# zhengyk19/vit-rpe-rope

Measured on AMD Instinct MI355X. Metric: train images/sec, CIFAR-10 ViT d=192 L=6 H=6, higher is better.
Workload: dtype bf16; 1 GPU; CIFAR-10-shaped 32x32 patch4 ViT d=192 L=6 H=6, --pos_encoding rope-axial theta=100, bf16, full train step (fwd+CE+bwd+AdamW), random-init weights; per_gpu_batch=512, global_batch=512, parallelism=dp1, hip_graph=True

## Files before the change

include/vitpe.h:

```cpp
#ifndef VITPE_H
#define VITPE_H

#ifdef __cplusplus
extern "C" {
#endif

#define VITPE_F32 0
#define VITPE_BF16 1

#define VITPE_PE_NONE 0
#define VITPE_PE_ABSOLUTE 1
#define VITPE_PE_RELATIVE 2
#define VITPE_PE_POLYNOMIAL 3
#define VITPE_PE_ROPE_AXIAL 4
#define VITPE_PE_ROPE_MIXED 5

#define VITPE_EPI_BIAS 0
#define VITPE_EPI_BIAS_GELU 1
#define VITPE_EPI_BIAS_RESID 2
#define VITPE_EPI_PATCH 3
#define VITPE_EPI_GELU_BWD 4

typedef void* vitpe_stream_t;

int vitpe_abi_version(void);

int vitpe_fused_attention_supported(int dtype, int N, int D, int HD);
int vitpe_pack_qkv_weights(int dtype, const float* wqkv, void* packed, int D, int HD, vitpe_stream_t stream);
int vitpe_fused_attention_fwd(int dtype, const void* xn, const void* wqkv, void* out, int B, int N,
                              int D, int HD, int mode, const float* cos, const float* sin,
                              const float* table, const float* coeff, int grid, int degree,
                              int coeff_per_head, vitpe_stream_t stream);
int vitpe_fused_attention_fwd_ln(int dtype, const void* x, const float* gamma, const float* beta,
                                 const float* mean, const float* rstd, void* xn_out, const void* wqkv,
                                 void* out, int B, int N, int D, int HD, int mode, const float* cos,
                                 const float* sin, const float* table, const float* coeff, int grid,
                                 int degree, int coeff_per_head, vitpe_stream_t stream);
int vitpe_fused_attention_wide_supported(int dtype, int N, int D, int HD);
int vitpe_qkv_wide_pack_elems(int D);
int vitpe_pack_qkv_weights_wide(int dtype, const float* wqkv, void* packed, int D, int HD, vitpe_stream_t stream);
int vitpe_fused_attention_fwd_wide(int dtype, const void* x, const float* gamma, const float* beta,
                                   const float* mean, const float* rstd, void* xn_out, const void* wqkv_wide,
                                   void* out, int B, int N, int D, int HD, int mode, const float* cos,
                                   const float* sin, const float* table, const float* coeff, int grid, int degree,
                                   int coeff_per_head, vitpe_stream_t stream);
int vitpe_fused_attention_bwd(int dtype, const void* xn, const void* wqkv, const void* dout,
                              void* dqkv, int B, int N, int D, int HD, int mode, const float* cos,
                              const float* sin, const float* table, const float* coeff, int grid,
                              int degree, int coeff_per_head, float* dtable, float* dcoeff,
                              float* dfreqs, vitpe_stream_t stream);
int vitpe_fused_attention_bwd_ln(int dtype, const void* x, const float* gamma, const float* beta,
                                 const float* mean, const float* rstd, const void* wqkv, const void* dout,
                                 void* dqkv, int B, int N, int D, int HD, int mode, const float* cos,
                                 const float* sin, const float* table, const float* coeff, int grid,
                                 int degree, int coeff_per_head, float* dtable, float* dcoeff,
                                 float* dfreqs, vitpe_stream_t stream);

int vitpe_attention_core_supported(int dtype, int N, int HD);
int vitpe_attention_core_fwd(int dtype, const void* qkv, void* out, int B, int N, int H, int HD, int mode,
                             const float* cos, const float* sin, const float* table, const float* coeff,
                             int grid, int degree, int coeff_per_head, vitpe_stream_t stream);
int vitpe_attention_core_bwd(int dtype, const void* qkv, const void* dout, void* dqkv, int B, int N, int H,
                             int HD, int mode, const float* cos, const float* sin, const float* table,
                             const float* coeff, int grid, int degree, int coeff_per_head, float* dtable,
                             float* dcoeff, float* dfreqs, vitpe_stream_t stream);
int vitpe_attention_core_bwd_tables(int dtype, const void* qkv, const void* dout, void* dqkv, int B, int N, int H,
                                    int HD, int mode, const float* cos, const float* sin, const float* table,
                                    const float* coeff, int grid, int degree, int coeff_per_head, float* dtable,
                                    float* dcoeff, float* dfreqs, float* dcos, float* dsin, float* workspace,
                                    vitpe_stream_t stream);
int vitpe_attention_fused64_supported(int dtype, int N, int H, int HD);
int vitpe_attention_fused64_fwd(int dtype, const void* xn, const void* wqkv_packed, void* qkv_out, void* out, int B,
                                int N, int H, int HD, int mode, const float* cos, const float* sin,
                                const float* table, const float* coeff, int grid, int degree, int coeff_per_head,
                                vitpe_stream_t stream);

int vitpe_philox4x32_10(const unsigned int* key2, const unsigned int* ctr4, unsigned int* out4);
int vitpe_dropout_mask(int site, const unsigned long long* rng, unsigned char* mask, long long n, int B, int H, int N,
                       float p, vitpe_stream_t stream);
int vitpe_dropout_fwd(int dtype, const void* x, const void* resid, void* y, long long n, const unsigned long long* rng,
                      float p, vitpe_stream_t stream);
int vitpe_dropout_bwd(int dtype, const void* dy, void* dx, long long n, const unsigned long long* rng, float p,
                      vitpe_stream_t stream);
int vitpe_drop_path_fwd(int dtype, const void* x, const void* resid, void* y, int B, long long per,
                        const unsigned long long* rng, float p, vitpe_stream_t stream);
int vitpe_drop_path_bwd(int dtype, const void* dy, void* dx, int B, long long per, const unsigned long long* rng, float p,
                        vitpe_stream_t stream);
int vitpe_attention_core_fwd_drop(int dtype, const void* qkv, void* out, int B, int N, int H, int HD, int mode,
                                  const float* cos, const float* sin, const float* table, const float* coeff,
                                  int grid, int degree, int coeff_per_head, const unsigned long long* rng, float p,
                                  vitpe_stream_t stream);
int vitpe_attention_core_bwd_drop(int dtype, const void* qkv, const void* dout, void* dqkv, int B, int N, int H,
                                  int HD, int mode, const float* cos, const float* sin, const float* table,
                                  const float* coeff, int grid, int degree, int coeff_per_head, float* dtable,
                                  float* dcoeff, float* dfreqs, const unsigned long long* rng, float p,
                                  vitpe_stream_t stream);

int vitpe_gemm_nt(int dtype, int epi, const void* A, const void* W, void* C, const float* bias,
                  const void* R, void* U, const float* ape, const float* cls, int M, int N, int K,
                  int P, int Ntok, vitpe_stream_t stream);
int vitpe_linear(int dtype, int epi, const void* A, const void* W, void* C, const float* bias,
                 const void* R, void* U, float* mean_out, float* rstd_out, float eps, int M, int N,
                 int K, vitpe_stream_t stream);
int vitpe_linear_ln(int dtype, int epi, const void* X, const float* gamma, const float* beta,
                    const float* mean, const float* rstd, void* xn_out, const void* W, void* C,
                    const float* bias, void* U, int M, int N, int K, vitpe_stream_t stream);
int vitpe_linear_lnbwd(int dtype, const void* dY, const void* Wt, void* dx, const void* x, const float* mean,
                       const float* rstd, const float* gamma, const void* dres, float* dgamma, float* dbeta,
                       int M, int K, vitpe_stream_t stream);
int vitpe_linear_lnbwd2(int dtype, const void* dY, const void* Wt_packed, void* dx, const void* x, const float* mean,
                        const float* rstd, const float* gamma, const void* dres, float* dgamma, float* dbeta, int M,
                        int K, vitpe_stream_t stream);
int vitpe_pack_weight_frags(int dtype, const float* W, void* packed, int R, int C, int kchunk, int phi,
                            vitpe_stream_t stream);
int vitpe_block_tail2_supported(int dtype, int D, int HID);
int vitpe_block_tail2_fwd(int dtype, const void* attn_out, const void* x_in, const void* Wp_packed, const float* bp,
                          const float* gamma, const float* beta, void* x_mid, float* mean2, float* rstd2,
                          void* xn_out, const void* W1_packed, const float* b1, const void* W2_packed,
                          const float* b2, void* gp_out, void* h_out, void* out, float* mean_out, float* rstd_out,
                          float eps2, float eps_next, int M, int D, int HID, vitpe_stream_t stream);
int vitpe_block_tail2_bwd(int dtype, const void* dy, const void* gp, const void* W2t_packed, const void* W1t_packed,
                          const void* x_mid, const float* mean2, const float* rstd2, const float* gamma, void* du,
                          void* dx_mid, float* dgamma, float* dbeta, const void* WpT_packed, void* da, int M, int D,
                          int HID, vitpe_stream_t stream);
int vitpe_block_tail2_bwd_pre(int dtype, const void* d_qkv, const void* WqT_packed, const void* x1, const float* mean1,
                              const float* rstd1, const float* gamma1, const void* dres1, float* dgamma1, float* dbeta1,
                              int K1, void* dy_out, const void* gp, const void* W2t_packed, const void* W1t_packed,
                              const void* x_mid, const float* mean2, const float* rstd2, const float* gamma, void* du,
                              void* dx_mid, float* dgamma, float* dbeta, const void* WpT_packed, void* da, int M, int D,
                              int HID, vitpe_stream_t stream);
int vitpe_gemm_tn(int dtype, const void* dY, const void* X, float* dW, float* dbias, int M, int N,
                  int K, int splits, vitpe_stream_t stream);

typedef struct {
  const void* dY;
  const void* X;
  float* dW;
  float* dbias;
  int M, N, K;
  int x_op;
  const float* x_mean;
  const float* x_rstd;
  const float* x_gamma;
  const float* x_beta;
} vitpe_wgrad_problem;
#define VITPE_XOP_NONE 0
#define VITPE_XOP_LAYERNORM 1
int vitpe_wgrad_group(int dtype, const vitpe_wgrad_problem* problems, int nprob, vitpe_stream_t stream);

int vitpe_layernorm_fwd(int dtype, const void* x, const float* gamma, const float* beta, void* y,
                        float* mean, float* rstd, int M, int D, float eps, vitpe_stream_t stream);
int vitpe_layernorm_bwd_blocks(int M);
int vitpe_layernorm_bwd(int dtype, const void* dy, const void* x, const float* mean,
                        const float* rstd, const float* gamma, const void* dres, void* dx,
                        float* dgamma, float* dbeta, float* workspace, int M, int D,
                        vitpe_stream_t stream);
int vitpe_reduce_partials(const float* partial, int nparts, int len0, int len1, float* dst0,
                          float* dst1, vitpe_stream_t stream);

int vitpe_resize_coeffs(int in, int out, int* bounds, int* kk, int ksize_cap);
int vitpe_resize_u8_supported(int S0, int S);
int vitpe_resize_u8(const unsigned char* src, unsigned char* dst, long long planes, int S0, int S,
                    const int* bounds_h, const int* kk_h, const int* bounds_v, const int* kk_v, int ksize,
                    vitpe_stream_t stream);

int vitpe_unfold(int dtype, const float* img, void* patches, int B, int C, int S, int p,
                 vitpe_stream_t stream);
int vitpe_unfold_u8(int dtype, const unsigned char* data, const long long* index, const float* mean,
                    const float* stdv, void* patches, float* img_out, int B, int C, int S, int p,
                    vitpe_stream_t stream);
int vitpe_patch_embed_supported(int dtype, int C, int S, int p, int D);
int vitpe_patch_embed(int dtype, const float* img, const unsigned char* data, const long long* index,
                      const float* nmean, const float* nstd, const void* W, const float* bias, const float* cls,
                      const float* ape, void* tokens, void* patches, float* mean, float* rstd, int B, int C, int S,
                      int p, int D, float eps, vitpe_stream_t stream);
int vitpe_embed_bwd(int dtype, const void* dtok, float* dcls, float* dape, void* dpatch, int B,
                    int Ntok, int D, vitpe_stream_t stream);

int vitpe_relative_position_index(long long* out, int L, vitpe_stream_t stream);
int vitpe_l1_distance_matrix(long long* out, int G, vitpe_stream_t stream);
int vitpe_rope_axial_tables(const float* inv_freq, float* cosv, float* sinv, int G, int half,
                            vitpe_stream_t stream);
int vitpe_rope_mixed_tables(const float* freqs, float* cosv, float* sinv, int H, int G, int half,
                            vitpe_stream_t stream);
int vitpe_relative_bias(const float* table, float* out, int H, int L, vitpe_stream_t stream);
int vitpe_polynomial_bias(const float* coeff, float* out, int H, int G, int degree, int per_head,
                          vitpe_stream_t stream);
int vitpe_relative_bias_bwd(const float* dbias, float* dtable, int H, int L, vitpe_stream_t stream);
int vitpe_polynomial_bias_bwd(const float* dbias, float* dcoeff, int H, int G, int degree, int per_head,
                              vitpe_stream_t stream);
int vitpe_rope_mixed_tables_bwd(const float* freqs, const float* dcos, const float* dsin, float* dfreqs, int H,
                                int G, int half, vitpe_stream_t stream);
int vitpe_apply_rotary(const float* x, float* y, const float* cosv, const float* sinv, int B, int H,
                       int P, int HD, int per_head, vitpe_stream_t stream);
int vitpe_apply_rotary_bwd(const float* dy, const float* x, const float* cosv, const float* sinv, float* dx,
                           float* dcos, float* dsin, float* workspace, int B, int H, int P, int HD, int per_head,
                           vitpe_stream_t stream);

int vitpe_head_fwd(int dtype, const void* x, const float* gamma, const float* beta, const float* Wh,
                   const float* bh, float* logits, float* ws_xhat, float* ws_yn, float* ws_rstd,
                   int B, int Ntok, int D, int Cn, float eps, vitpe_stream_t stream);
int vitpe_cross_entropy(const float* logits, const long long* labels, float* dlogits, float* out2,
                        int B, int Cn, float grad_scale, vitpe_stream_t stream);
int vitpe_cross_entropy_ctl(const float* logits, const long long* labels, float* dlogits, float* out2,
                            float* metric_acc, const float* ctl, int B, int Cn, vitpe_stream_t stream);
int vitpe_head_bwd(int dtype, const float* dlogits, const float* Wh, const float* gamma,
                   const float* ws_xhat, const float* ws_yn, const float* ws_rstd, float* ws_dyn,
                   void* dx, float* dWh, float* dbh, float* dgamma, float* dbeta, int B, int Ntok,
                   int D, int Cn, vitpe_stream_t stream);
int vitpe_head_loss(int dtype, const void* x, const float* gamma, const float* beta, const float* Wh,
                    const float* bh, const long long* labels, float* logits, float* dlogits, float* ws_xhat,
                    float* ws_yn, float* ws_dyn, void* dx, float* out2, float* metric_acc, float* scratch,
                    float* dWh, float* dbh, float* dgamma, float* dbeta, int B, int Ntok, int D, int Cn,
                    float eps, float grad_scale, vitpe_stream_t stream);

int vitpe_head_step(int dtype, const void* x, const float* gamma, const float* beta, const float* Wh,
                    const float* bh, const long long* labels, float* logits, float* dlogits, float* ws_xhat,
                    float* ws_yn, float* ws_dyn, void* dx, float* out2, float* metric_acc, float* per_image,
                    const float* ctl, float* dWh, float* dbh, float* dgamma, float* dbeta, int B, int Ntok,
                    int D, int Cn, float eps, float* hp_tick, vitpe_stream_t stream);

int vitpe_adamw_step(float* p, float* g, float* m, float* v, void* shadow_bf16, float* hp,
                     long long n, int zero_grad, vitpe_stream_t stream);
int vitpe_cast(int dtype, const float* src, void* dst, long long n, vitpe_stream_t stream);
int vitpe_transpose_cast(int dtype, const float* src, void* dst, int R, int C, vitpe_stream_t stream);
int vitpe_refresh_shadows(int dtype, const float* flat, void* dst_base, const void* desc, int ndesc,
                          int total_tiles, const unsigned short* tile_map, vitpe_stream_t stream);


#ifdef __cplusplus
}
#endif
#endif
```

vit-rpe-rope_amd/csrc/wgrad.hip:

```cpp
#include "common.h"
#include <stdlib.h>

namespace vitpe {

constexpr int WG_MAXPROB = 28;
constexpr int WG_BLK = 192;

struct WgProb {
  const void* dY;
  const void* X;
  float* dW;
  float* dbias;
  const float* xmean;
  const float* xrstd;
  const float* xgamma;
  const float* xbeta;
  int M, N, K;
  int xop;
  int unit0;
  int nbn;
  int stages;
};
constexpr int WG_TABLE = 512;
struct WgArgs {
  int nprob, total_units, units_per_wg;
  int use_table;
  int nranges;
  int full_rounds, total_blocks;
  int tail_rounds;
  int bk;
  int range_major;
  unsigned long long* census;
  WgProb p[WG_MAXPROB];
  unsigned short table[WG_TABLE];
};
static_assert(sizeof(WgArgs) <= 4096, "kernel argument block");
constexpr int WG_CENSUS_STAGES = 24, WG_CENSUS_SLOTS = 4;

template <typename T> struct WgLayout;
template <> struct WgLayout<bf16> {
  static constexpr int LD = WG_BLK;
  static __device__ __forceinline__ int chunk(int r, int cc) {
    const int s = ((r >> 1) & 1) | (((r >> 3) & 1) << 1);
    return r * LD + ((((cc >> 1) ^ s)) << 4) + ((cc & 1) << 3);
  }
  static __device__ __forceinline__ Frag<bf16> tr(const bf16* tile, int rb0, int rb1, int c0) { return tr_ld<LD>(tile, rb0, rb1, c0); }
  template <int LD>
  static __device__ __forceinline__ Frag<bf16> tr_ld(const bf16* tile, int rb0, int rb1, int c0) {
    const int i = threadIdx.x & 15, q = i >> 2, p = i & 3;
    typedef __attribute__((address_space(3))) s16x4 lds_s16x4;
    const int r0 = rb0 + q, r1 = rb1 + q;
    constexpr int PAR = (LD % 128 == 0) ? 4 : 0;
    const int s0 = (((r0 >> 1) & 1) | (((r0 >> 3) & 1) << 1)) ^ ((r0 & 1) * PAR), s1 = (((r1 >> 1) & 1) | (((r1 >> 3) & 1) << 1)) ^ ((r1 & 1) * PAR);
    const bf16* a0 = tile + r0 * LD + (((c0 >> 4) ^ s0) << 4) + 4 * p;
    const bf16* a1 = tile + r1 * LD + (((c0 >> 4) ^ s1) << 4) + 4 * p;
    s16x4 lo = __builtin_amdgcn_ds_read_tr16_b64_v4i16((lds_s16x4*)a0);
    s16x4 hi = __builtin_amdgcn_ds_read_tr16_b64_v4i16((lds_s16x4*)a1);
    const s16x8 both = __builtin_shufflevector(lo, hi, 0, 1, 2, 3, 4, 5, 6, 7);
    Frag<bf16> f;
    f.v = __builtin_bit_cast(bf16x8, both);
    return f;
  }
};
template <> struct WgLayout<float> {
  static constexpr int LD = WG_BLK + 4;
  static __device__ __forceinline__ int chunk(int r, int cc) { return r * LD + cc * 4; }
  static __device__ __forceinline__ Frag<float> tr(const float* tile, int rb0, int rb1, int c0) {
    return ld_frag_tr(tile, LD, rb0, rb1, c0);
  }
};

template <class RunFn>
VITPE_DEV void wg_dispatch(const WgArgs& a, RunFn run) {
  if (a.use_table == 2) {
    const int G = gridDim.x, idx = (blockIdx.x & 7) * (G >> 3) + (blockIdx.x >> 3);
    const int nrounds = a.range_major ? a.full_rounds : a.full_rounds + a.tail_rounds;
    for (int r = 0; r < nrounds; ++r) {
      int gb, rng = 0, R = 1;
      if (a.range_major) {
        const int vb = r * G + idx;
        R = a.nranges;
        rng = vb / a.total_blocks;
        gb = rng < R ? vb - rng * a.total_blocks : a.total_blocks;
      } else if (r < a.full_rounds) {
        gb = r * G + idx;
      } else {
        R = a.nranges;
        const int rem = a.total_blocks - a.full_rounds * G, q = (r - a.full_rounds) * G + idx;
        if (q >= rem * R) continue;
        rng = q / rem;
        gb = a.full_rounds * G + q % rem;
      }
      if (gb >= a.total_blocks) continue;
      int pi = 0, b0 = 0;
      for (int i = 0; i < a.nprob; ++i) {
        const int nb = a.p[i].nbn * ((a.p[i].K + a.bk - 1) / a.bk);
        if (gb >= b0 + nb) { b0 += nb; pi = i + 1; } else break;
      }
      const WgProb& P = a.p[pi];
      const int spr = (P.stages + R - 1) / R;
      const int ub = P.unit0 + (gb - b0) * P.stages;
      const int u0 = ub + min(P.stages, rng * spr), uend = ub + min(P.stages, (rng + 1) * spr);
      if (u0 < uend) run(u0, uend);
    }
    return;
  }
  int u0, uend;
  if (a.use_table == 1) {
    const unsigned ent = a.table[blockIdx.x];
    if (ent == 0xFFFFu) return;
    const WgProb& P = a.p[ent >> 11];
    const int blk = (int)((ent >> 5) & 0x3Fu), rng = (int)(ent & 0x1Fu);
    const int spr = (P.stages + a.nranges - 1) / a.nranges;
    u0 = P.unit0 + blk * P.stages + min(P.stages, rng * spr);
    uend = P.unit0 + blk * P.stages + min(P.stages, (rng + 1) * spr);
  } else {
    u0 = blockIdx.x * a.units_per_wg;
    uend = min(a.total_units, u0 + a.units_per_wg);
  }
  if (u0 >= uend) return;
  run(u0, uend);
}

template <typename T, bool CENSUS, bool LNX>
__global__ __launch_bounds__(768) void wgrad_group_kernel(WgArgs a) {
  using LY = WgLayout<T>;
  constexpr int RPS = 128 / (int)sizeof(T);
  constexpr int CPS = RPS / 32;
  constexpr int CHN = CH<T>::n;
  constexpr int CPR = WG_BLK / CHN;
  static_assert(RPS * CPR == 2 * 768, "a slab is two chunks per thread");
  constexpr int SLAB = RPS * LY::LD;
  __shared__ __attribute__((aligned(16))) T sm[2 * 2 * SLAB];

  const int tid = threadIdx.x, lane = tid & 63, c = lane & 15, g = lane >> 4;
  const int wave = __builtin_amdgcn_readfirstlane(tid >> 6);
  const int wn = wave / 3, wk = wave % 3;

  struct Cur {
    const T* dY; const T* X; float* dW; float* dbias;
    const float* xmean; const float* xrstd; const float* xgamma; const float* xbeta;
    int M, N, K, n0, k0, stage, stages, xop;
  };
  auto decode = [&](int u, Cur& s) {
    int pi = 0;
    for (int i = 1; i < a.nprob; ++i) pi = (u >= a.p[i].unit0) ? i : pi;
    const WgProb& P = a.p[pi];
    const int ub = u - P.unit0, blk = ub / P.stages;
    s.dY = reinterpret_cast<const T*>(P.dY); s.X = reinterpret_cast<const T*>(P.X); s.dW = P.dW; s.dbias = P.dbias;
    s.M = P.M; s.N = P.N; s.K = P.K; s.stages = P.stages;
    s.xmean = P.xop ? P.xmean : reinterpret_cast<const float*>(P.dY);
    s.xrstd = P.xop ? P.xrstd : reinterpret_cast<const float*>(P.dY);
    s.xgamma = P.xgamma; s.xbeta = P.xbeta; s.xop = P.xop;
    s.stage = ub - blk * P.stages;
    s.n0 = (blk % P.nbn) * WG_BLK;
    s.k0 = (blk / P.nbn) * a.bk;
  };

  const Chunk16 zero = {0u, 0u, 0u, 0u};
  Chunk16 rg[4];
  float lnA[2], lnB[2];
  bool ln_staged = false;
  auto gload = [&](const Cur& s) {
    const int mb = s.stage * RPS;
    ln_staged = LNX && s.xop == 1;
#pragma unroll
    for (int i = 0; i < 4; ++i) {
      const int q = tid + 768 * (i & 1), row = q / CPR, cc = q % CPR;
      const int gm = mb + row;
      if (i < 2) {
        const int gn = s.n0 + cc * CHN;
        rg[i] = (gm < s.M && gn < s.N) ? *reinterpret_cast<const Chunk16*>(s.dY + (size_t)gm * s.N + gn) : zero;
      } else {
        const int gk = s.k0 + cc * CHN;
        const bool ok = gm < s.M && gk < s.K;
        rg[i] = ok ? *reinterpret_cast<const Chunk16*>(s.X + (size_t)gm * s.K + gk) : zero;
        if (LNX) {
          const int gs = (s.xop == 1) ? min(gm, s.M - 1) : 0;
          lnA[i - 2] = s.xrstd[gs];
          lnB[i - 2] = s.xmean[gs];
        }
      }
    }
  };
  auto sstore = [&](int buf) {
#pragma unroll
    for (int i = 0; i < 4; ++i) {
      const int q = tid + 768 * (i & 1), row = q / CPR, cc = q % CPR;
      Chunk16 v = rg[i];
      if (LNX && i >= 2 && ln_staged) {
        float f[CHN];
        chunk_to_f32<T>(v, f);
        const float rs = lnA[i - 2], nb = -lnB[i - 2] * rs;
#pragma unroll
        for (int t = 0; t < CHN; ++t) f[t] = fmaf(f[t], rs, nb);
        v = f32_to_chunk<T>(f);
      }
      *reinterpret_cast<Chunk16*>(sm + (buf * 2 + (i >> 1)) * SLAB + LY::chunk(row, cc)) = v;
    }
  };

  f32x4 acc[3][4], accb[3];
  auto clear = [&]() {
#pragma unroll
    for (int nt = 0; nt < 3; ++nt) {
      accb[nt] = (f32x4){0.f, 0.f, 0.f, 0.f};
#pragma unroll
      for (int kt = 0; kt < 4; ++kt) acc[nt][kt] = (f32x4){0.f, 0.f, 0.f, 0.f};
    }
  };
  Frag<T> ones;
#pragma unroll
  for (int t = 0; t < 8; ++t) ones.v[t] = from_f32<T>(1.0f);

  auto compute = [&](int buf, bool bias) {
    const T* sY = sm + (buf * 2 + 0) * SLAB;
    const T* sX = sm + (buf * 2 + 1) * SLAB;
#pragma unroll
    for (int cs = 0; cs < CPS; ++cs) {
      const int rb0 = cs * 32 + 8 * g, rb1 = rb0 + 4;
      Frag<T> fy[3], fx[4];
#pragma unroll
      for (int nt = 0; nt < 3; ++nt) fy[nt] = LY::tr(sY, rb0, rb1, wn * 48 + 16 * nt);
#pragma unroll
      for (int kt = 0; kt < 4; ++kt) fx[kt] = LY::tr(sX, rb0, rb1, wk * 64 + 16 * kt);
#pragma unroll
      for (int nt = 0; nt < 3; ++nt)
#pragma unroll
        for (int kt = 0; kt < 4; ++kt) mma(fy[nt], fx[kt], acc[nt][kt]);
      if (bias) {
#pragma unroll
        for (int nt = 0; nt < 3; ++nt) mma(fy[nt], ones, accb[nt]);
      }
    }
  };
  auto flush = [&](const Cur& s, bool bias) {
    float gam[4], bet[4];
#pragma unroll
    for (int kt = 0; kt < 4; ++kt) {
      const int gk = s.k0 + wk * 64 + 16 * kt + c;
      gam[kt] = (LNX && s.xop == 1 && gk < s.K) ? s.xgamma[gk] : 1.f;
      bet[kt] = (LNX && s.xop == 1 && gk < s.K) ? s.xbeta[gk] : 0.f;
    }
#pragma unroll
    for (int nt = 0; nt < 3; ++nt)
#pragma unroll
      for (int r = 0; r < 4; ++r) {
        const int gn = s.n0 + wn * 48 + 16 * nt + 4 * g + r;
#pragma unroll
        for (int kt = 0; kt < 4; ++kt) {
          const int gk = s.k0 + wk * 64 + 16 * kt + c;
          float v = acc[nt][kt][r];
          if (LNX && s.xop == 1) v = fmaf(v, gam[kt], bet[kt] * accb[nt][r]);
          if (gn < s.N && gk < s.K) atomicAdd(s.dW + (size_t)gn * s.K + gk, v);
        }
        if (bias && c == 0 && gn < s.N) atomicAdd(s.dbias + gn, accb[nt][r]);
      }
    clear();
  };

  bool first_run = true;
  auto run = [&](int u0, int uend) {
    if (!first_run) __syncthreads();
    first_run = false;
  Cur cur, nxt;
    decode(u0, cur);
    gload(cur);
    clear();
    auto stamp = [&](int u, int slot) {
      if (CENSUS && lane == 0 && u - u0 < WG_CENSUS_STAGES)
        a.census[(((size_t)blockIdx.x * 12 + wave) * WG_CENSUS_STAGES + (u - u0)) * WG_CENSUS_SLOTS + slot] = __builtin_amdgcn_s_memtime();
    };
    for (int u = u0; u < uend; ++u) {
      const int buf = (u - u0) & 1;
      sstore(buf);
      stamp(u, 0);
      nxt = cur;
      bool flush_now = (u + 1 == uend);
      if (u + 1 < uend) {
        if (cur.stage + 1 < cur.stages) nxt.stage = cur.stage + 1;
        else { decode(u + 1, nxt); flush_now = true; }
        gload(nxt);
      }
      stamp(u, 2);
      __syncthreads();
      stamp(u, 1);
      const bool bias = (cur.dbias != nullptr) && cur.k0 == 0 && wk == 0;
      compute(buf, bias || (LNX && cur.xop == 1));
      stamp(u, 3);
      if (flush_now) flush(cur, bias);
      cur = nxt;
    }
  };

  wg_dispatch(a, run);
}

constexpr int WW_BK = 384, WW_TH = 512;

__global__ __launch_bounds__(WW_TH) void wgrad_wide_kernel(WgArgs a) {
  using T = bf16;
  using LY = WgLayout<bf16>;
  constexpr int RPS = 64, YLD = WG_BLK, XLD = WW_BK;
  constexpr int YSLAB = RPS * YLD, XSLAB = RPS * XLD, STG = YSLAB + XSLAB;
  constexpr int YI = YSLAB / 512, XI = XSLAB / 512, NI = (YI + XI) / 8;
  static_assert((YI + XI) % 8 == 0, "instructions per wave");
  __shared__ __attribute__((aligned(1024))) T sm[2 * STG];

  const int tid = threadIdx.x, lane = tid & 63, c = lane & 15, g = lane >> 4;
  const int wave = __builtin_amdgcn_readfirstlane(tid >> 6);
  const int wn = wave >> 2, wk = wave & 3;

  struct Cur { const T* dY; const T* X; float* dW; float* dbias; int M, N, K, n0, k0, stage, stages; };
  auto decode = [&](int u, Cur& s) {
    int pi = 0;
    for (int i = 1; i < a.nprob; ++i) pi = (u >= a.p[i].unit0) ? i : pi;
    const WgProb& P = a.p[pi];
    const int ub = u - P.unit0, blk = ub / P.stages;
    s.dY = reinterpret_cast<const T*>(P.dY); s.X = reinterpret_cast<const T*>(P.X); s.dW = P.dW; s.dbias = P.dbias;
    s.M = P.M; s.N = P.N; s.K = P.K; s.stages = P.stages;
    s.stage = ub - blk * P.stages;
    s.n0 = (blk % P.nbn) * WG_BLK;
    s.k0 = (blk / P.nbn) * WW_BK;
  };
  auto swz = [](int r, int cl) { return ((((cl >> 1) ^ (((r >> 1) & 1) | (((r >> 3) & 1) << 1))) << 1) | (cl & 1)); };
  auto swzx = [](int r, int cl) {
    return ((((cl >> 1) ^ ((((r >> 1) & 1) | (((r >> 3) & 1) << 1)) ^ ((r & 1) << 2))) << 1) | (cl & 1));
  };
  static_assert(YI == 24 && XI == 48, "instruction j of a wave: j < 3 -> dY slab, else X slab");
  const unsigned sm_lds = (unsigned)(uintptr_t)(__attribute__((address_space(3))) void*)sm;
  auto dma = [&](const Cur& s, int buf) {
    const int mb = s.stage * RPS;
    int ln = lane;
    asm volatile("" : "+v"(ln));
#pragma unroll
    for (int j = 0; j < NI; ++j) {
      const int q = wave + 8 * j;
      const T* src;
      if (j < 3) {
        const int p = q * 64 + ln, r = p / (YLD / 8), cl = p % (YLD / 8);
        src = s.dY + (size_t)min(mb + r, s.M - 1) * s.N + s.n0 + swz(r, cl) * 8;
      } else {
        const int p = (q - YI) * 64 + ln, r = p / (XLD / 8), cl = p % (XLD / 8);
        src = s.X + (size_t)min(mb + r, s.M - 1) * s.K + s.k0 + swzx(r, cl) * 8;
      }
      const unsigned dst = sm_lds + (unsigned)(buf * STG + q * 512) * 2;
      unsigned keep;
      asm volatile("s_mov_b32 %0, m0\n\ts_mov_b32 m0, %2\n\ts_nop 0\n\tglobal_load_lds_dwordx4 %1, off\n\ts_mov_b32 m0, %0"
                   : "=&s"(keep) : "v"(src), "s"(dst) : "memory");
    }
  };

  f32x4 acc[6][6], accb[2];
  auto clear = [&]() {
    accb[0] = accb[1] = (f32x4){0.f, 0.f, 0.f, 0.f};
#pragma unroll
    for (int nt = 0; nt < 6; ++nt)
#pragma unroll
      for (int kt = 0; kt < 6; ++kt) acc[nt][kt] = (f32x4){0.f, 0.f, 0.f, 0.f};
  };
  Frag<T> ones;
#pragma unroll
  for (int t = 0; t < 8; ++t) ones.v[t] = from_f32<T>(1.0f);

  auto compute = [&](int buf, bool bias) {
    const T* sY = sm + buf * STG;
    const T* sX = sY + YSLAB;
#pragma unroll
    for (int cs = 0; cs < 2; ++cs) {
      const int rb0 = cs * 32 + 8 * g, rb1 = rb0 + 4;
      __builtin_amdgcn_sched_barrier(0);
      Frag<T> fy[6];
#pragma unroll
      for (int nt = 0; nt < 6; ++nt) fy[nt] = LY::tr_ld<YLD>(sY, rb0, rb1, wn * 96 + 16 * nt);
#pragma unroll
      for (int h = 0; h < 2; ++h) {
        Frag<T> fx[3];
#pragma unroll
        for (int t = 0; t < 3; ++t) fx[t] = LY::tr_ld<XLD>(sX, rb0, rb1, wk * 96 + 16 * (3 * h + t));
#pragma unroll
        for (int nt = 0; nt < 6; ++nt)
#pragma unroll
          for (int t = 0; t < 3; ++t) mma(fy[nt], fx[t], acc[nt][3 * h + t]);
        __builtin_amdgcn_sched_barrier(0);
      }
      if (bias) {
        if (wk == 0) { mma(fy[0], ones, accb[0]); mma(fy[1], ones, accb[1]); }
        else if (wk == 1) { mma(fy[2], ones, accb[0]); mma(fy[3], ones, accb[1]); }
        else { mma(fy[4], ones, accb[0]); mma(fy[5], ones, accb[1]); }
      }
    }
  };
  auto flush = [&](const Cur& s, bool bias) {
#pragma unroll
    for (int nt = 0; nt < 6; ++nt)
#pragma unroll
      for (int r = 0; r < 4; ++r) {
        const int gn = s.n0 + wn * 96 + 16 * nt + 4 * g + r;
        float* row = s.dW + (size_t)gn * s.K + s.k0 + wk * 96 + c;
#pragma unroll
        for (int kt = 0; kt < 6; ++kt) atomicAdd(row + 16 * kt, acc[nt][kt][r]);
      }
    if (bias && c == 0) {
#pragma unroll
      for (int t = 0; t < 2; ++t)
#pragma unroll
        for (int r = 0; r < 4; ++r) atomicAdd(s.dbias + s.n0 + wn * 96 + 16 * (2 * wk + t) + 4 * g + r, accb[t][r]);
    }
    clear();
  };

  bool first_run = true;
  auto run = [&](int u0, int uend) {
    if (!first_run) __syncthreads();
    first_run = false;
    Cur cur, nxt;
    decode(u0, cur);
    dma(cur, 0);
    clear();
    for (int u = u0; u < uend; ++u) {
      const int buf = (u - u0) & 1;
      __builtin_amdgcn_s_waitcnt(0x0F70);
      __syncthreads();
      if (cur.stage * RPS + RPS > cur.M) {
        const int first = cur.M - cur.stage * RPS;
        T* sY = sm + buf * STG;
        for (int q = tid; q < (RPS - first) * (YLD / 8); q += WW_TH)
          *reinterpret_cast<Chunk16*>(sY + first * YLD + q * 8) = (Chunk16){0u, 0u, 0u, 0u};
        __syncthreads();
      }
      nxt = cur;
      bool flush_now = (u + 1 == uend);
      if (u + 1 < uend) {
        if (cur.stage + 1 < cur.stages) nxt.stage = cur.stage + 1;
        else { decode(u + 1, nxt); flush_now = true; }
        dma(nxt, buf ^ 1);
      }
      const bool bias = (cur.dbias != nullptr) && cur.k0 == 0 && wk < 3;
      compute(buf, bias);
      if (flush_now) flush(cur, bias);
      cur = nxt;
    }
  };
  wg_dispatch(a, run);
}

}

using namespace vitpe;

struct vitpe_wgrad_problem_abi {
  const void* dY;
  const void* X;
  float* dW;
  float* dbias;
  int M, N, K, x_op;
  const float* x_mean;
  const float* x_rstd;
  const float* x_gamma;
  const float* x_beta;
};

static int wgrad_cu_count() {
  static int n = 0;
  if (n == 0) {
    int dev = 0, v = 0;
    if (hipGetDevice(&dev) != hipSuccess || hipDeviceGetAttribute(&v, hipDeviceAttributeMultiprocessorCount, dev) != hipSuccess || v <= 0)
      v = 256;
    n = v;
  }
  return n;
}

static int wgrad_group_launch(int dtype, const void* problems, int nprob, unsigned long long* census, hipStream_t stream);
static bool g_wide_ok = true;
extern "C" int vitpe_debug_set_wgrad_wide(int on) { g_wide_ok = on != 0; return 0; }

extern "C" int vitpe_wgrad_group(int dtype, const void* problems, int nprob, hipStream_t stream) {
  return wgrad_group_launch(dtype, problems, nprob, nullptr, stream);
}

extern "C" int vitpe_debug_wgrad_census(int dtype, const void* problems, int nprob, unsigned long long* census,
                                        hipStream_t stream) {
  VITPE_REQUIRE(census != nullptr && dtype == 1);
  return wgrad_group_launch(dtype, problems, nprob, census, stream);
}

static int wgrad_group_launch(int dtype, const void* problems, int nprob, unsigned long long* census, hipStream_t stream) {
  VITPE_REQUIRE(problems && nprob >= 0 && nprob <= WG_MAXPROB && (dtype == 0 || dtype == 1));
  const vitpe_wgrad_problem_abi* pr = reinterpret_cast<const vitpe_wgrad_problem_abi*>(problems);
  const int RPS = dtype == 1 ? 64 : 32, CHN = dtype == 1 ? 8 : 4;
  WgArgs a{};
  a.census = census;
  bool wide = g_wide_ok && dtype == 1 && census == nullptr && nprob > 0;
  for (int i = 0; i < nprob; ++i)
    wide = wide && (pr[i].M == 0 || (pr[i].x_op == 0 && pr[i].N % WG_BLK == 0 && pr[i].K % WW_BK == 0));
  a.bk = wide ? WW_BK : WG_BLK;
  int units = 0, np = 0;
  for (int i = 0; i < nprob; ++i) {
    const vitpe_wgrad_problem_abi& p = pr[i];
    VITPE_REQUIRE(p.dY && p.X && p.dW && p.M >= 0 && p.N > 0 && p.K > 0 && p.N % CHN == 0 && p.K % CHN == 0);
    if (p.M == 0) continue;
    WgProb& q = a.p[np++];
    VITPE_REQUIRE(p.x_op == 0 || (p.x_op == 1 && p.x_mean && p.x_rstd && p.x_gamma && p.x_beta));
    q.dY = p.dY; q.X = p.X; q.dW = p.dW; q.dbias = p.dbias; q.M = p.M; q.N = p.N; q.K = p.K;
    q.xop = p.x_op; q.xmean = p.x_mean; q.xrstd = p.x_rstd; q.xgamma = p.x_gamma; q.xbeta = p.x_beta;
    q.unit0 = units;
    q.nbn = (p.N + WG_BLK - 1) / WG_BLK;
    q.stages = (p.M + RPS - 1) / RPS;
    const long long nu = (long long)q.nbn * ((p.K + a.bk - 1) / a.bk) * q.stages;
    VITPE_REQUIRE(units + nu < (1LL << 30));
    units += (int)nu;
  }
  if (units == 0) return 0;
  a.nprob = np;
  a.total_units = units;
  const int ncu = wgrad_cu_count();
  int grid = 0;
  int total_blocks = 0, max_blocks = 0, min_stages = 1 << 30;
  for (int i = 0; i < np; ++i) {
    const int nb = a.p[i].nbn * ((a.p[i].K + a.bk - 1) / a.bk);
    total_blocks += nb;
    max_blocks = nb > max_blocks ? nb : max_blocks;
    min_stages = a.p[i].stages < min_stages ? a.p[i].stages : min_stages;
  }
  int R = (2 * ncu) / (total_blocks > 0 ? total_blocks : 1);
  if (R > 255) R = 255;
  if (R >= 2 && R <= 8 && R <= min_stages / 4 && max_blocks <= 63 && np <= 31) {
    int len[8] = {0, 0, 0, 0, 0, 0, 0, 0};
    bool fits = true;
    for (int i = 0; i < WG_TABLE; ++i) a.table[i] = 0xFFFFu;
    for (int r = 0; r < R && fits; ++r)
      for (int i = 0; i < np && fits; ++i) {
        const int nb = a.p[i].nbn * ((a.p[i].K + a.bk - 1) / a.bk);
        int x = 0;
        for (int k = 1; k < 8; ++k) x = len[k] < len[x] ? k : x;
        for (int b = 0; b < nb; ++b) {
          const int id = (len[x] + b) * 8 + x;
          if (id >= WG_TABLE) { fits = false; break; }
          a.table[id] = (unsigned short)(((unsigned)i << 11) | ((unsigned)b << 5) | (unsigned)r);
        }
        len[x] += nb;
      }
    if (fits) {
      int mx = 0;
      for (int k = 0; k < 8; ++k) mx = len[k] > mx ? len[k] : mx;
      a.use_table = 1;
      a.nranges = R;
      grid = mx * 8;
    }
  }
  const int G = ncu & ~7;
  if (!a.use_table && G >= 8 && total_blocks >= G) {
    a.use_table = 2;
    a.total_blocks = total_blocks;
    a.full_rounds = total_blocks / G;
    const int rem = total_blocks - a.full_rounds * G;
    int bestR = 1, bestT = rem > 0 ? 1 : 0;
    int Rmax = min_stages / 4;
    if (Rmax > 8) Rmax = 8;
    for (int Rc = 2; rem > 0 && Rc <= Rmax; ++Rc) {
      const int Tc = (rem * Rc + G - 1) / G;
      if ((long long)Tc * bestR < (long long)bestT * Rc) { bestR = Rc; bestT = Tc; }
    }
    a.nranges = bestR;
    a.tail_rounds = bestT;
    grid = G;
  }
  if (!a.use_table && G >= 8 && total_blocks > 0 && total_blocks < G) {
    int bestR = 0, bestk = 0;
    double besteff = 0.0;
    for (int k = 1; k <= 3; ++k) {
      int Rk = (k * G) / total_blocks;
      if (Rk > min_stages / 4) Rk = min_stages / 4;
      if (Rk > 31) Rk = 31;
      if (Rk < 2) continue;
      const double eff = (double)total_blocks * Rk / (double)(((total_blocks * Rk + G - 1) / G) * G);
      if (eff > besteff + 1e-9) { besteff = eff; bestR = Rk; bestk = k; }
    }
    if (bestR >= 2 && besteff >= 0.97) {
      a.use_table = 2;
      a.range_major = 1;
      a.total_blocks = total_blocks;
      a.nranges = bestR;
      a.full_rounds = (total_blocks * bestR + G - 1) / G;
      grid = G;
      (void)bestk;
    }
  }
  if (!a.use_table) {
    const int wgs = units < ncu ? units : ncu;
    a.units_per_wg = (units + wgs - 1) / wgs;
    grid = (units + a.units_per_wg - 1) / a.units_per_wg;
  }
  bool lnx = false;
  for (int i = 0; i < np; ++i) lnx = lnx || a.p[i].xop != 0;
  if (census != nullptr) VITPE_REQUIRE(!lnx && dtype == 1);
  if (wide) hipLaunchKernelGGL(wgrad_wide_kernel, dim3(grid), dim3(WW_TH), 0, stream, a);
  else if (census != nullptr) hipLaunchKernelGGL((wgrad_group_kernel<bf16, true, false>), dim3(grid), dim3(768), 0, stream, a);
  else if (dtype == 1 && lnx) hipLaunchKernelGGL((wgrad_group_kernel<bf16, false, true>), dim3(grid), dim3(768), 0, stream, a);
  else if (dtype == 1) hipLaunchKernelGGL((wgrad_group_kernel<bf16, false, false>), dim3(grid), dim3(768), 0, stream, a);
  else if (lnx) hipLaunchKernelGGL((wgrad_group_kernel<float, false, true>), dim3(grid), dim3(768), 0, stream, a);
  else hipLaunchKernelGGL((wgrad_group_kernel<float, false, false>), dim3(grid), dim3(768), 0, stream, a);
  VITPE_CHECK_LAUNCH();
}
```

vit-rpe-rope_amd/vitpe/engine.py:

```python
from __future__ import annotations

import math
import os
from typing import Dict, List, Optional

import torch
import torch.distributed as dist
import torch.nn as nn

from . import _lib as L
from . import ddp
from . import kernels as K
from .positional_encoding import (AbsolutePositionalEncoding, PolynomialRPE, RelativePositionalEncoding, RoPEAxial,
                                  RoPEMixed)
from .vit import VisionTransformer

ALIGN = 8


def engine_unsupported(model):
    active = []
    for blk in model.blocks:
        if blk.attn.qkv.bias is not None:
            active.append("qkv_bias")
        if blk.attn.attn_drop_p > 0.:
            active.append("attn_drop")
        if blk.attn.proj_drop_p > 0. or blk.mlp.drop > 0.:
            active.append("drop")
        if blk.drop_path_p > 0.:
            active.append("drop_path")
    return sorted(set(active))


class TrainEngine:
    def __init__(self, model: VisionTransformer, batch_size: int, compute_dtype=torch.bfloat16, lr=1e-3,
                 weight_decay=0.01, betas=(0.9, 0.999), eps=1e-8, process_group=None, use_graph=True, fuse_ln=None):
        active = engine_unsupported(model)
        if active:
            raise NotImplementedError("TrainEngine does not support " + ", ".join(active) + " (the fused training path has "
                                      "no qkv bias and no dropout); train this model through the module path instead")
        dev = next(model.parameters()).device
        if dev.type != "cuda":
            raise L.VitpeError("TrainEngine needs the model on the HIP device (no CPU path)")
        self.model, self.dev, self.T, self.B = model, dev, compute_dtype, batch_size
        self.pg = process_group
        self.world = dist.get_world_size(process_group) if (dist.is_available() and dist.is_initialized()) else 1
        self.use_graph = use_graph
        m = model
        ok = m.embed_dim == 192
        if fuse_ln is None and "VITPE_FUSE_LN" in os.environ:
            fuse_ln = {"fwd": "fwd", "all": True, "off": False}[os.environ["VITPE_FUSE_LN"]]
        self.fuse_ln = ok and fuse_ln is not False
        self.fuse_ln_bwd = ok and (fuse_ln is True or fuse_ln is None)
        self.D, self.H, self.Lyr = m.embed_dim, m.num_heads, len(m.blocks)
        self.p = m.patch_size
        self.C = m.patch_embed.weight.shape[1]

        self.P = m.num_patches
        self.N = self.P + 1
        self.grid = int(math.sqrt(self.P))
        self.S = self.grid * self.p
        self.fuse_embed = (os.environ.get("VITPE_FUSE_EMBED", "1") == "1" and
                           K.patch_embed_supported(compute_dtype, self.C, self.S, self.p, self.D))
        self.hid = m.blocks[0].mlp.fc1.weight.shape[0]
        self.Cn = m.num_classes
        self.M = self.B * self.N
        self.attn_fused = K.fused_attention_supported(self.T, self.N, self.D, self.D // self.H)
        if not self.attn_fused and not K.attention_core_supported(self.T, self.N, self.D // self.H):
            raise L.VitpeError(f"no attention kernel for N={self.N}, D={self.D}, hd={self.D // self.H}")
        self._save_hidden = True
        self.attn_wide = (self.attn_fused and K.fused_attention_wide_supported(self.T, self.N, self.D, self.D // self.H)
                          and os.environ.get("VITPE_ATTN_WIDE", "1") == "1")
        self.attn_fused64 = (not self.attn_fused and os.environ.get("VITPE_ATTN_FUSED64", "1") == "1"
                             and K.attention_fused64_supported(self.T, self.N, self.H, self.D // self.H))
        if not self.attn_fused:
            self.fuse_ln = self.fuse_ln_bwd = False
        self.tail2 = (self.fuse_ln and self.fuse_ln_bwd and os.environ.get("VITPE_TAIL2", "1") == "1"
                      and K.block_tail2_supported(self.T, self.D, self.hid))
        self.lnbwd2 = self.tail2 and os.environ.get("VITPE_LNBWD2", "1") == "1"
        self.fuse_lnbwd = self.lnbwd2 and os.environ.get("VITPE_FUSE_LNBWD", "1") == "1"
        self._build_flat(lr, weight_decay, betas, eps)
        self._build_buffers()
        self.split_layer = max(1, self.Lyr // 2)
        self.bucket_off = self._off[id(next(self.model.blocks[self.split_layer].parameters()))] \
            if self.Lyr >= 2 else 0
        self.overlap_comm = self.world > 1 and self.Lyr >= 2
        self.allpairs = (ddp.AllPairsSum(self.pg) if self.world > 1 and os.environ.get("VITPE_DDP_ALLPAIRS", "0") == "1"
                         else None)
        self._comm_stream = torch.cuda.Stream(device=dev) if self.allpairs is not None else None
        self.ddp_graph = self.world > 1 and os.environ.get("VITPE_DDP_GRAPH", "0") == "1"
        self.graph_fb = self.graph_fb2 = self.graph_opt = None
        self.steps_done = 0

    def _build_flat(self, lr, wd, betas, eps):
        params = list(self.model.parameters())
        starts, n = ddp.flat_layout([prm.numel() for prm in params], ALIGN)
        offs = {id(prm): o for prm, o in zip(params, starts)}
        self.n_flat = n
        f = dict(dtype=torch.float32, device=self.dev)
        self.flat_p, self.flat_g = torch.zeros(n, **f), torch.zeros(n, **f)
        self.flat_m, self.flat_v = torch.zeros(n, **f), torch.zeros(n, **f)
        self.flat_s = torch.zeros(n, dtype=torch.bfloat16, device=self.dev) if self.T == torch.bfloat16 else None
        self._off = offs
        for prm in params:
            o = offs[id(prm)]
            view = self.flat_p[o:o + prm.numel()].view(prm.shape)
            view.copy_(prm.data)
            prm.data = view
            prm.grad = self.flat_g[o:o + prm.numel()].view(prm.shape)
        self.model.register_load_state_dict_post_hook(lambda _m, _keys: self.sync_from_model())
        self.hp = torch.zeros(16, **f)
        self.hp[:5] = torch.tensor([lr, betas[0], betas[1], eps, wd], **f)
        self.hp[8] = 1.0 / self.world
        self._st: Dict[int, torch.Tensor] = {}
        self._pk: Dict[int, torch.Tensor] = {}
        self._pkw: Dict[int, torch.Tensor] = {}
        self._fr: Dict[int, torch.Tensor] = {}
        self._frt: Dict[int, torch.Tensor] = {}
        self._gemm_weights: List[nn.Parameter] = []
        recs, off, tile0 = [], 0, 0
        def alloc(w):
            nonlocal off
            o = off
            off += (w.numel() + ALIGN - 1) // ALIGN * ALIGN
            return o
        def add(w, kind, hd, kind2=-1, hd2=0):
            nonlocal tile0
            R, C = w.shape
            o1 = alloc(w)
            o2 = alloc(w) if kind2 >= 0 else 0
            recs.append((self._off[id(w)], o1, o2, R, C, tile0, kind, hd, kind2, hd2, 0))
            tile0 += ((R + 31) // 32) * ((C + 31) // 32)
            spans.append((w, kind, o1))
            if kind2 >= 0:
                spans.append((w, kind2, o2))
        spans = []
        HDh = self.D // self.H
        gen2 = self.tail2
        for blk in self.model.blocks:
            qkv, proj, fc1, fc2 = blk.attn.qkv.weight, blk.attn.proj.weight, blk.mlp.fc1.weight, blk.mlp.fc2.weight
            self._gemm_weights += [qkv, proj, fc1, fc2]
            if self.attn_fused:
                add(qkv, 1, HDh, *((4, 64) if self.lnbwd2 else (0, 0)))
                if self.attn_wide:
                    add(qkv, 6, HDh)
            else:
                add(qkv, 0, 0, *((2, 64) if self.attn_fused64 else ()))
            if self.tail2:
                add(proj, 2, 192, *((5, 192) if gen2 else (0, 0)))
                add(fc1, 3, 192, *((5, 32) if gen2 else (0, 0)))
                add(fc2, 3, 32, *((5, 192) if gen2 else (0, 0)))
            else:
                for w in (proj, fc1, fc2):
                    add(w, 0, 0)
        self._shadow_flat = torch.empty(off, dtype=self.T, device=self.dev)
        for w, kind, o in spans:
            R, C = w.shape
            if kind == 0:
                self._st[id(w)] = self._shadow_flat[o:o + R * C].view(C, R)
            elif kind == 1:
                self._pk[id(w)] = self._shadow_flat[o:o + R * C].view(R, C)
            elif kind == 6:
                self._pkw[id(w)] = self._shadow_flat[o:o + R * C]
            elif kind < 4:
                self._fr[id(w)] = self._shadow_flat[o:o + R * C].view(R, C)
            else:
                self._frt[id(w)] = self._shadow_flat[o:o + R * C].view(C, R)
        import numpy as np
        rec = np.zeros(len(recs), dtype=np.dtype([("src", "<i8"), ("dst", "<i8"), ("dst2", "<i8"), ("R", "<i4"), ("C", "<i4"),
                                                   ("tile0", "<i4"), ("kind", "<i4"), ("HD", "<i4"), ("kind2", "<i4"),
                                                   ("HD2", "<i4"), ("pad", "<i4")]))
        for i, r in enumerate(recs):
            rec[i] = r
        self._desc = torch.from_numpy(rec.view(np.uint8).copy()).to(self.dev)
        self._ndesc, self._ntiles = len(recs), tile0
        tmap = np.zeros(tile0, dtype=np.int16)
        for i, r in enumerate(recs):
            tmap[r[5]:] = i
        self._tile_map = torch.from_numpy(tmap).to(self.dev)
        self.refresh_shadows()

    def Pm(self, prm):
        return prm.data

    def Gr(self, prm):
        o = self._off[id(prm)]
        return self.flat_g[o:o + prm.numel()].view(prm.shape)

    def Sh(self, prm):
        if self.T == torch.float32:
            return prm.data
        o = self._off[id(prm)]
        return self.flat_s[o:o + prm.numel()].view(prm.shape)

    def St(self, prm):
        return self._st[id(prm)]

    def Pk(self, prm):
        return self._pk[id(prm)]

    def Pkw(self, prm):
        return self._pkw[id(prm)]

    def _attn_fwd(self, x, blk, out, ln=None, xn_out=None):
        if self.attn_wide:
            return K.fused_attention_fwd_wide(x, self.Pkw(blk.attn.qkv.weight), self.H, self.pe, out=out, ln=ln, xn_out=xn_out)
        return K.fused_attention_fwd(x, self.Pk(blk.attn.qkv.weight), self.H, self.pe, out=out, ln=ln, xn_out=xn_out)

    def _attn_layer_fwd(self, l, save_qkv=True):
        blk, a = self.model.blocks[l], self.act[l]
        if self.fuse_ln:
            return self._attn_fwd(self.x[l], blk, a["a"], ln=(blk.norm1.weight.data, blk.norm1.bias.data, a["m1"], a["r1"]),
                                  xn_out=a["xn1"])
        if self.attn_fused:
            return self._attn_fwd(a["xn1"], blk, a["a"])
        if self.attn_fused64:
            return K.attention_fused64_fwd(a["xn1"], self.Fr(blk.attn.qkv.weight), self.H, self.pe,
                                           qkv_out=(self.qkv_l[l] if save_qkv else None), out=a["a"])
        return K.attention_core_fwd(self.qkv_l[l], self.H, self.pe, out=a["a"])

    def _attn_bwd(self, l, dout):
        blk, a = self.model.blocks[l], self.act[l]
        if not self.attn_fused:
            return K.attention_core_bwd(self.qkv_l[l], dout, self.H, self.pe, out=self.dqkv_l[l], **self.pe_grads)
        if self.recompute_ln:
            return K.fused_attention_bwd(self.x[l], self.Pk(blk.attn.qkv.weight), dout, self.H, self.pe, out=self.dqkv_l[l],
                                         ln=(blk.norm1.weight.data, blk.norm1.bias.data, a["m1"], a["r1"]), **self.pe_grads)
        return K.fused_attention_bwd(a["xn1"], self.Pk(blk.attn.qkv.weight), dout, self.H, self.pe, out=self.dqkv_l[l],
                                     **self.pe_grads)

    def Fr(self, prm):
        return self._fr[id(prm)]

    def Frt(self, prm):
        return self._frt[id(prm)]

    def refresh_shadows(self, cast_flat=True):
        if self.T == torch.bfloat16 and cast_flat:
            K.cast(self.flat_p, torch.bfloat16, out=self.flat_s)
        K.refresh_shadows(self.flat_p, self._shadow_flat, self._desc, self._ndesc, self._ntiles, self._tile_map)

    def set_lr(self, lr: float):
        self.hp[0] = lr

    def _build_buffers(self):
        B, N, D, M, T, dev = self.B, self.N, self.D, self.M, self.T, self.dev
        e = lambda *s, dt=T: torch.empty(*s, dtype=dt, device=dev)
        f = lambda *s: torch.empty(*s, dtype=torch.float32, device=dev)
        self.images = f(B, self.C, self.S, self.S)
        self.labels = torch.zeros(B, dtype=torch.int64, device=dev)
        self.patches = e(B * self.P, self.C * self.p * self.p)
        self.x = [e(B, N, D) for _ in range(self.Lyr + 1)]
        self.group_wgrad = os.environ.get("VITPE_GROUP_WGRAD", "1") == "1"
        self.recompute_ln = (self.attn_fused and self.fuse_ln and self.fuse_ln_bwd and self.tail2
                             and self.group_wgrad and os.environ.get("VITPE_RECOMPUTE_LN", "0") == "1")
        xn = (lambda: None) if self.recompute_ln else (lambda: e(B, N, D))
        self.act = []
        for _ in range(self.Lyr):
            self.act.append(dict(xn1=xn(), m1=f(M), r1=f(M), a=e(B, N, D), xmid=e(B, N, D), xn2=xn(),
                                 m2=f(M), r2=f(M), h=e(M, self.hid), u=e(M, self.hid)))
        self.logits, self.dlogits = f(B, self.Cn), f(B, self.Cn)
        self.out2 = f(2)
        self.metric_acc = torch.zeros(2, dtype=torch.float32, device=dev)
        self.ce_ctl = torch.zeros(4, dtype=torch.float32, device=dev)
        self._valid = None
        self.set_valid(B)
        self.head_scratch = torch.zeros(2 * B, dtype=torch.float32, device=dev)
        self.fuse_head = self.Cn <= 64 and self.D <= 768 and os.environ.get("VITPE_FUSE_HEAD", "1") == "1"
        self.head_ws = (f(B, D), f(B, D), f(B))
        self.ws_dyn = f(B, D)
        self.dtmp = e(B, N, D)
        self.dx_out = [e(B, N, D) for _ in range(self.Lyr + 1)]
        self.dx_out[self.Lyr].zero_()
        self.dx_mid = [e(B, N, D) for _ in range(self.Lyr)]
        self.du_l = [e(M, self.hid) for _ in range(self.Lyr)]
        self.dqkv_l = [e(B, N, 3 * D) for _ in range(self.Lyr)]
        self.qkv_l = [] if self.attn_fused else [e(B, N, 3 * D) for _ in range(self.Lyr)]
        self.dqkv, self.du = self.dqkv_l[0], self.du_l[0]
        self.dataset, self.batch_idx = None, None
        self._wg_groups = {}
        self.dpatch = e(B * self.P, D)
        self.ln_ws = K.layernorm_bwd_workspace(M, D, dev)
        pe = self.model.pos_embed
        mode = self.model.pos_encoding_type
        self.pe = K.PETables(mode if mode != "absolute" else "none", self.grid)
        self.pe_grads = dict(dtable=None, dcoeff=None, dfreqs=None)
        if isinstance(pe, RelativePositionalEncoding):
            self.pe.table = pe.relative_position_bias_table.data
            self.pe_grads["dtable"] = self.Gr(pe.relative_position_bias_table)
        elif isinstance(pe, PolynomialRPE):
            self.pe.coeff, self.pe.degree = pe.coefficients.data, pe.degree
            self.pe.coeff_per_head = not pe.shared_across_heads
            self.pe_grads["dcoeff"] = self.Gr(pe.coefficients)
        elif isinstance(pe, RoPEAxial):
            self.pe.cos, self.pe.sin = K.rope_axial_tables(pe.inv_freq.contiguous(), self.grid)
        elif isinstance(pe, RoPEMixed):
            self.pe.cos, self.pe.sin = K.rope_mixed_tables(pe.freqs.data, self.grid)
            self.pe_grads["dfreqs"] = self.Gr(pe.freqs)

    def _forward(self, head=True, save=False):
        self._save_hidden = save
        mdl, B, N, D, M = self.model, self.B, self.N, self.D, self.M
        ape = mdl.pos_embed.pos_embed.data[0, :self.P] if isinstance(mdl.pos_embed, AbsolutePositionalEncoding) else None
        if self.fuse_embed:
            src = (dict(data=self.dataset.images, index=self.batch_idx, mean=self.dataset.mean, std=self.dataset.std)
                   if self.dataset is not None else dict(images=self.images))
            b0 = mdl.blocks[0]
            K.patch_embed(self.Sh(mdl.patch_embed.weight).view(D, -1), mdl.patch_embed.bias.data, mdl.cls_token.data.view(-1),
                          ape, self.p, self.T, out=self.x[0], patches_out=self.patches,
                          stats=(self.act[0]["m1"], self.act[0]["r1"]) if self.fuse_ln else None, eps=b0.norm1.eps, **src)
        else:
            if self.dataset is not None:
                K.unfold_u8(self.dataset.images, self.batch_idx, self.dataset.mean, self.dataset.std, self.p, self.T,
                            out=self.patches)
            else:
                K.unfold(self.images, self.p, self.T, out=self.patches)
            K.patch_embed_gemm(self.patches, self.Sh(mdl.patch_embed.weight).view(D, -1), mdl.patch_embed.bias.data,
                               mdl.cls_token.data.view(-1), ape, B, self.P, out=self.x[0])
            if self.fuse_ln:
                b0 = mdl.blocks[0]
                K.layernorm_fwd(self.x[0], b0.norm1.weight.data, b0.norm1.bias.data, b0.norm1.eps, mean=self.act[0]["m1"],
                                rstd=self.act[0]["r1"], stats_only=True)
        if isinstance(mdl.pos_embed, RoPEMixed):
            K.rope_mixed_tables(mdl.pos_embed.freqs.data, self.grid, self.pe.cos, self.pe.sin)
        for l, blk in enumerate(mdl.blocks):
            a, xin = self.act[l], self.x[l]
            if self.fuse_ln:
                self._attn_layer_fwd(l)
                nxt = (self.act[l + 1]["m1"], self.act[l + 1]["r1"]) if l + 1 < self.Lyr else None
                eps_next = mdl.blocks[min(l + 1, self.Lyr - 1)].norm1.eps
                if self.tail2:
                    self._block_tail_fwd(l, blk, a, nxt)
                    continue
                K.linear(a["a"].view(M, D), self.Sh(blk.attn.proj.weight), blk.attn.proj.bias.data,
                         epi=L.EPI_BIAS_RESID, resid=xin.view(M, D), out=a["xmid"].view(M, D), stats=(a["m2"], a["r2"]),
                         eps=blk.norm2.eps)
                K.linear_ln(a["xmid"].view(M, D), blk.norm2.weight.data, blk.norm2.bias.data, a["m2"], a["r2"],
                            self.Sh(blk.mlp.fc1.weight), blk.mlp.fc1.bias.data, epi=L.EPI_BIAS_GELU, u=a["u"], out=a["h"],
                            xn_out=a["xn2"].view(M, D))
                K.linear(a["h"], self.Sh(blk.mlp.fc2.weight), blk.mlp.fc2.bias.data, epi=L.EPI_BIAS_RESID,
                         resid=a["xmid"].view(M, D), out=self.x[l + 1].view(M, D), stats=nxt, eps=eps_next)
                continue
            K.layernorm_fwd(xin, blk.norm1.weight.data, blk.norm1.bias.data, blk.norm1.eps, out=a["xn1"],
                            mean=a["m1"], rstd=a["r1"])
            if not self.attn_fused and not self.attn_fused64:
                K.linear(a["xn1"].view(M, D), self.Sh(blk.attn.qkv.weight), None, out=self.qkv_l[l].view(M, 3 * D))
            self._attn_layer_fwd(l, save_qkv=self._save_hidden)
            K.linear(a["a"].view(M, D), self.Sh(blk.attn.proj.weight), blk.attn.proj.bias.data, epi=L.EPI_BIAS_RESID,
                     resid=xin.view(M, D), out=a["xmid"].view(M, D))
            K.layernorm_fwd(a["xmid"], blk.norm2.weight.data, blk.norm2.bias.data, blk.norm2.eps, out=a["xn2"],
                            mean=a["m2"], rstd=a["r2"])
            K.linear(a["xn2"].view(M, D), self.Sh(blk.mlp.fc1.weight), blk.mlp.fc1.bias.data, epi=L.EPI_BIAS_GELU,
                     u=a["u"], out=a["h"])
            K.linear(a["h"], self.Sh(blk.mlp.fc2.weight), blk.mlp.fc2.bias.data, epi=L.EPI_BIAS_RESID,
                     resid=a["xmid"].view(M, D), out=self.x[l + 1].view(M, D))
        if head:
            K.head_fwd(self.x[-1], mdl.norm.weight.data, mdl.norm.bias.data, mdl.head.weight.data, mdl.head.bias.data,
                       mdl.norm.eps, save=True, logits=self.logits, ws=self.head_ws)

    def _block_tail_fwd(self, l, blk, a, nxt, save=None):
        M, D = self.M, self.D
        eps_next = self.model.blocks[min(l + 1, self.Lyr - 1)].norm1.eps
        if save is None:
            save = self._save_hidden
        K.block_tail2_fwd(a["a"].view(M, D), self.x[l].view(M, D), self.Fr(blk.attn.proj.weight),
                          blk.attn.proj.bias.data, blk.norm2.weight.data, blk.norm2.bias.data,
                          self.Fr(blk.mlp.fc1.weight), blk.mlp.fc1.bias.data, self.Fr(blk.mlp.fc2.weight),
                          blk.mlp.fc2.bias.data, x_mid=a["xmid"].view(M, D), mean2=a["m2"], rstd2=a["r2"],
                          xn_out=(a["xn2"].view(M, D) if (save and not self.recompute_ln) else None),
                          gp=(a["u"].view(torch.float16) if save else None), h=(a["h"] if save else None), out=self.x[l + 1].view(M, D),
                          stats=nxt, eps2=blk.norm2.eps, eps_next=eps_next, save=save)

    def _block_tail_bwd(self, l, blk, a, pre=False):
        M, D, G = self.M, self.D, self.Gr
        if pre:
            up, ua = self.model.blocks[l + 1], self.act[l + 1]
            K.block_tail2_bwd_pre(self.dqkv_l[l + 1].view(M, 3 * D), self.Frt(up.attn.qkv.weight), self.x[l + 1].view(M, D),
                                  ua["m1"], ua["r1"], up.norm1.weight.data, self.dx_mid[l + 1].view(M, D), G(up.norm1.weight),
                                  G(up.norm1.bias), self.dx_out[l + 1].view(M, D), a["u"].view(torch.float16), self.Frt(blk.mlp.fc2.weight),
                                  self.Frt(blk.mlp.fc1.weight), a["xmid"].view(M, D), a["m2"], a["r2"], blk.norm2.weight.data,
                                  G(blk.norm2.weight), G(blk.norm2.bias), self.Frt(blk.attn.proj.weight), du=self.du_l[l],
                                  out=self.dx_mid[l].view(M, D), da=self.dtmp.view(M, D))
            return
        K.block_tail2_bwd(self.dx_out[l + 1].view(M, D), a["u"].view(torch.float16), self.Frt(blk.mlp.fc2.weight),
                          self.Frt(blk.mlp.fc1.weight), a["xmid"].view(M, D), a["m2"], a["r2"], blk.norm2.weight.data,
                          G(blk.norm2.weight), G(blk.norm2.bias), self.Frt(blk.attn.proj.weight), du=self.du_l[l],
                          out=self.dx_mid[l].view(M, D), da=self.dtmp.view(M, D))

    def _tail_bytes(self, fwd: bool) -> int:
        M, D, hid, es = self.M, self.D, self.hid, 2 if self.T == torch.bfloat16 else 4
        if fwd:
            return ((4 if self.recompute_ln else 5) * M * D + 2 * M * hid) * es
        return (4 * M * D + 2 * M * hid) * es

    def _fwd_train(self):
        self._forward(head=not self.fuse_head, save=True)

    def _loss(self, tick=True):
        self._ticked = bool(tick and self.fuse_head)
        if self.fuse_head:
            mdl, G = self.model, self.Gr
            K.head_step(self.x[-1], mdl.norm.weight.data, mdl.norm.bias.data, mdl.head.weight.data, mdl.head.bias.data,
                        self.labels, self.logits, self.dlogits, self.head_ws, self.ws_dyn, self.dx_out[self.Lyr], self.out2,
                        self.metric_acc, self.head_scratch, self.ce_ctl, G(mdl.head.weight), G(mdl.head.bias),
                        G(mdl.norm.weight), G(mdl.norm.bias), eps=mdl.norm.eps, hp_tick=(self.hp if tick else None))
            return
        K.cross_entropy_ctl(self.logits, self.labels, self.ce_ctl, dlogits=self.dlogits, out2=self.out2,
                            metric_acc=self.metric_acc)

    def _wgrad_problems(self, lo, hi, with_embed):
        mdl, D, M, G = self.model, self.D, self.M, self.Gr
        probs = []
        for l in range(hi, lo - 1, -1):
            blk, a = mdl.blocks[l], self.act[l]
            if self.recompute_ln:
                fc1 = (self.du_l[l], a["xmid"].view(M, D), G(blk.mlp.fc1.weight), G(blk.mlp.fc1.bias),
                       (a["m2"], a["r2"], blk.norm2.weight.data, blk.norm2.bias.data))
                qkv = (self.dqkv_l[l].view(M, 3 * D), self.x[l].view(M, D), G(blk.attn.qkv.weight), None,
                       (a["m1"], a["r1"], blk.norm1.weight.data, blk.norm1.bias.data))
            else:
                fc1 = (self.du_l[l], a["xn2"].view(M, D), G(blk.mlp.fc1.weight), G(blk.mlp.fc1.bias))
                qkv = (self.dqkv_l[l].view(M, 3 * D), a["xn1"].view(M, D), G(blk.attn.qkv.weight), None)
            probs += [(self.dx_out[l + 1].view(M, D), a["h"], G(blk.mlp.fc2.weight), G(blk.mlp.fc2.bias)), fc1,
                      (self.dx_mid[l].view(M, D), a["a"].view(M, D), G(blk.attn.proj.weight), G(blk.attn.proj.bias)), qkv]
        if with_embed:
            probs.append((self.dpatch, self.patches, G(mdl.patch_embed.weight).view(D, -1), G(mdl.patch_embed.bias)))
        return probs

    def _wgrad_group(self, part):
        if part not in self._wg_groups:
            hi, lo = self.Lyr - 1, 0
            if part == "upper":
                lo = self.split_layer
            elif part == "lower":
                hi = self.split_layer - 1
            probs = self._wgrad_problems(lo, hi, part != "upper")
            ng = -(-len(probs) // K.WgradGroup.MAX)
            per = -(-len(probs) // ng)
            self._wg_groups[part] = [K.WgradGroup(probs[i:i + per]) for i in range(0, len(probs), per)]
        for grp in self._wg_groups[part]:
            grp.launch()

    def _wgrad(self, fn):
        if not self.group_wgrad:
            fn()

    def _backward(self, part="all"):
        mdl, B, N, D, M = self.model, self.B, self.N, self.D, self.M
        G = self.Gr
        hi, lo = self.Lyr - 1, 0
        if part == "upper":
            lo = self.split_layer
        elif part == "lower":
            hi = self.split_layer - 1
        if part != "lower" and not self.fuse_head:
            dxL = self.dx_out[self.Lyr]
            K.head_bwd(self.dlogits, mdl.head.weight.data, mdl.norm.weight.data, self.head_ws, self.T, N,
                       G(mdl.head.weight), G(mdl.head.bias), G(mdl.norm.weight), G(mdl.norm.bias), dx=dxL,
                       ws_dyn=self.ws_dyn)
        for l in range(hi, lo - 1, -1):
            blk, a = mdl.blocks[l], self.act[l]
            dy3, dmid3, du, dqkv = self.dx_out[l + 1], self.dx_mid[l], self.du_l[l], self.dqkv_l[l]
            dy = dy3.view(M, D)
            self._wgrad(lambda: K.gemm_tn(dy, a["h"], G(blk.mlp.fc2.weight), G(blk.mlp.fc2.bias)))
            fc1_wgrad = lambda: K.gemm_tn(du, a["xn2"].view(M, D), G(blk.mlp.fc1.weight), G(blk.mlp.fc1.bias))
            tail_done = False
            if self.tail2:
                self._block_tail_bwd(l, blk, a, pre=(self.fuse_lnbwd and self.group_wgrad and l < hi))
                self._wgrad(fc1_wgrad)
                tail_done = True
            else:
                K.linear(dy, self.St(blk.mlp.fc2.weight), None, epi=L.EPI_GELU_BWD, u=a["u"], out=du)
                self._wgrad(fc1_wgrad)
                if self.fuse_ln_bwd:
                    K.linear_lnbwd(du, self.St(blk.mlp.fc1.weight), a["xmid"].view(M, D), a["m2"], a["r2"],
                                   blk.norm2.weight.data, dy, G(blk.norm2.weight), G(blk.norm2.bias),
                                   out=dmid3.view(M, D))
                else:
                    K.linear(du, self.St(blk.mlp.fc1.weight), None, out=self.dtmp.view(M, D))
                    K.layernorm_bwd(self.dtmp, a["xmid"], a["m2"], a["r2"], blk.norm2.weight.data, G(blk.norm2.weight),
                                    G(blk.norm2.bias), dres=dy3, out=dmid3, workspace=self.ln_ws)
            dm = dmid3.view(M, D)
            self._wgrad(lambda: K.gemm_tn(dm, a["a"].view(M, D), G(blk.attn.proj.weight), G(blk.attn.proj.bias)))
            if not tail_done:
                K.linear(dm, self.St(blk.attn.proj.weight), None, out=self.dtmp.view(M, D))
            self._attn_bwd(l, self.dtmp)
            self._wgrad(lambda: K.gemm_tn(dqkv.view(M, 3 * D), a["xn1"].view(M, D), G(blk.attn.qkv.weight), None))
            if self.fuse_lnbwd and self.group_wgrad and l > lo:
                pass
            elif self.fuse_ln_bwd and self.lnbwd2:
                K.linear_lnbwd2(dqkv.view(M, 3 * D), self.Frt(blk.attn.qkv.weight), self.x[l].view(M, D), a["m1"],
                                a["r1"], blk.norm1.weight.data, dm, G(blk.norm1.weight), G(blk.norm1.bias),
                                out=self.dx_out[l].view(M, D))
            elif self.fuse_ln_bwd:
                K.linear_lnbwd(dqkv.view(M, 3 * D), self.St(blk.attn.qkv.weight), self.x[l].view(M, D), a["m1"],
                               a["r1"], blk.norm1.weight.data, dm, G(blk.norm1.weight), G(blk.norm1.bias),
                               out=self.dx_out[l].view(M, D))
            else:
                K.linear(dqkv.view(M, 3 * D), self.St(blk.attn.qkv.weight), None, out=self.dtmp.view(M, D))
                K.layernorm_bwd(self.dtmp, self.x[l], a["m1"], a["r1"], blk.norm1.weight.data, G(blk.norm1.weight),
                                G(blk.norm1.bias), dres=dmid3, out=self.dx_out[l], workspace=self.ln_ws)
        if part != "upper":
            dape = None
            if isinstance(mdl.pos_embed, AbsolutePositionalEncoding):
                dape = G(mdl.pos_embed.pos_embed)[0, :self.P]
            K.embed_bwd(self.dx_out[0], G(mdl.cls_token).view(-1), dape, out=self.dpatch)
            if not self.group_wgrad:
                K.gemm_tn(self.dpatch, self.patches, G(mdl.patch_embed.weight).view(D, -1), G(mdl.patch_embed.bias))
        if self.group_wgrad:
            self._wgrad_group(part)

    def _optimizer(self):
        K.adamw_step(self.flat_p, self.flat_g, self.flat_m, self.flat_v, self.hp, shadow_bf16=self.flat_s, ticked=getattr(self, "_ticked", False),
                     zero_grad=True)
        self._ticked = False
        self.refresh_shadows(cast_flat=False)

    def _allreduce(self):
        if self.allpairs is not None:
            self.allpairs(self.flat_g)
        else:
            ddp.allreduce_sum_(self.flat_g, self.pg)

    def set_valid(self, n_valid: int, n_valid_global: Optional[int] = None):
        if n_valid_global is None:
            n_valid_global = n_valid * self.world
        if not (0 <= n_valid <= self.B and n_valid_global >= max(n_valid, 1)):
            raise L.VitpeError(f"set_valid({n_valid}, {n_valid_global}) with engine batch {self.B}")
        if self._valid != (n_valid, n_valid_global):
            self._valid = (n_valid, n_valid_global)
            host = torch.tensor([self.world / n_valid_global, 1.0 / n_valid_global, float(n_valid), 0.0])
            self.ce_ctl.copy_(host, non_blocking=False)

    def sync_from_model(self):
        self.refresh_shadows()

    def broadcast_parameters(self, src=0):
        if self.world > 1:
            ddp.broadcast_(self.flat_p, src, self.pg)
            self.refresh_shadows()

    def capture(self):
        snap = [t.clone() for t in (self.flat_p, self.flat_m, self.flat_v, self.hp, self.metric_acc)]
        s = torch.cuda.Stream()
        s.wait_stream(torch.cuda.current_stream())
        with torch.cuda.stream(s):
            for _ in range(2):
                self._fwd_train(); self._loss(); self._backward(); self._optimizer()
        torch.cuda.current_stream().wait_stream(s)
        torch.cuda.synchronize()
        for t, c in zip((self.flat_p, self.flat_m, self.flat_v, self.hp, self.metric_acc), snap):
            t.copy_(c)
        self.flat_g.zero_()
        self.refresh_shadows()
        torch.cuda.synchronize()
        if self.ddp_graph:
            try:
                g = torch.cuda.CUDAGraph()
                with torch.cuda.graph(g, capture_error_mode="thread_local"):
                    self._fwd_train(); self._loss()
                    if self.overlap_comm:
                        self._backward("upper")
                        side, main = torch.cuda.Stream(), torch.cuda.current_stream()
                        side.wait_stream(main)
                        with torch.cuda.stream(side):
                            dist.all_reduce(self.flat_g[self.bucket_off:], op=dist.ReduceOp.SUM, group=self.pg)
                        self._backward("lower")
                        dist.all_reduce(self.flat_g[:self.bucket_off], op=dist.ReduceOp.SUM, group=self.pg)
                        main.wait_stream(side)
                    else:
                        self._backward()
                        self._allreduce()
                    self._optimizer()
                torch.cuda.synchronize()
                self.graph_fb, self.graph_fb2, self.graph_opt = g, None, None
                return
            except Exception as exc:
                import warnings
                warnings.warn(f"VITPE_DDP_GRAPH: capturing the all-reduces failed ({exc!r}); using the host-stitched step")
                self.ddp_graph = False
                torch.cuda.synchronize()
                self.flat_g.zero_()
        self.graph_fb = torch.cuda.CUDAGraph()
        with torch.cuda.graph(self.graph_fb, capture_error_mode="thread_local"):
            self._fwd_train(); self._loss()
            if self.world == 1:
                self._backward(); self._optimizer()
            elif self.overlap_comm:
                self._backward("upper")
            else:
                self._backward()
        if self.world > 1:
            if self.overlap_comm:
                self.graph_fb2 = torch.cuda.CUDAGraph()
                with torch.cuda.graph(self.graph_fb2, capture_error_mode="thread_local"):
                    self._backward("lower")
            self.graph_opt = torch.cuda.CUDAGraph()
            with torch.cuda.graph(self.graph_opt, capture_error_mode="thread_local"):
                self._optimizer()
        torch.cuda.synchronize()

    def attach_dataset(self, dataset):
        if dataset is self.dataset:
            return
        if dataset is not None:
            C, S = dataset.images.shape[1], dataset.images.shape[2]
            if (C, S) != (self.C, self.S) or dataset.images.device != self.dev:
                raise L.VitpeError(f"dataset is {C}x{S}x{S} on {dataset.images.device}, engine expects "
                                   f"{self.C}x{self.S}x{self.S} on {self.dev}")
            if self.batch_idx is None:
                self.batch_idx = torch.zeros(self.B, dtype=torch.int64, device=self.dev)
        self.dataset = dataset
        self.graph_fb = self.graph_fb2 = self.graph_opt = None

    def _load_indices(self, idx: torch.Tensor, dataset=None):
        dataset = dataset if dataset is not None else self.dataset
        if dataset is None:
            raise L.VitpeError("no dataset attached (TrainEngine.attach_dataset)")
        n = idx.shape[0] if idx.dim() == 1 else -1
        if not (1 <= n <= self.B) or idx.dtype != torch.int64:
            raise L.VitpeError(f"expected 1..{self.B} int64 sample indices, got {tuple(idx.shape)} {idx.dtype}")
        if n < self.B:
            self.batch_idx.fill_(idx[0])
            self.batch_idx[:n].copy_(idx, non_blocking=True)
        else:
            self.batch_idx.copy_(idx, non_blocking=True)
        torch.index_select(dataset.labels, 0, self.batch_idx, out=self.labels)
        return n

    def step_indexed(self, idx: torch.Tensor, n_valid_global: Optional[int] = None, n_valid: Optional[int] = None):
        n = self._load_indices(idx)
        self.set_valid(n if n_valid is None else min(n, n_valid), n_valid_global)
        self.step()

    def forward_indexed(self, idx: torch.Tensor, dataset=None) -> torch.Tensor:
        keep = self.dataset
        if dataset is not None:
            if self.batch_idx is None:
                self.batch_idx = torch.zeros(self.B, dtype=torch.int64, device=self.dev)
            self.dataset = dataset
        try:
            n = self._load_indices(idx)
            self._forward()
        finally:
            self.dataset = keep
        return self.logits[:n]

    def _load_batch(self, images, labels):
        n = images.shape[0]
        if not (1 <= n <= self.B) or tuple(images.shape[1:]) != tuple(self.images.shape[1:]):
            raise L.VitpeError(f"engine was built for batches of up to {self.B} x {tuple(self.images.shape[1:])}, "
                               f"got {tuple(images.shape)}")
        if n < self.B:
            self.images.copy_(images[:1].expand_as(self.images))
            self.images[:n].copy_(images, non_blocking=True)
            if labels is not None:
                self.labels.fill_(0)
                self.labels[:n].copy_(labels, non_blocking=True)
        else:
            self.images.copy_(images, non_blocking=True)
            if labels is not None:
                self.labels.copy_(labels, non_blocking=True)
        return n

    def step(self, images: Optional[torch.Tensor] = None, labels: Optional[torch.Tensor] = None,
             n_valid_global: Optional[int] = None, exchange: bool = True):
        if images is not None:
            if self.dataset is not None:
                raise L.VitpeError("a resident dataset is attached: use step_indexed (or attach_dataset(None))")
            self.set_valid(self._load_batch(images, labels), n_valid_global)
        if self.use_graph:
            if self.graph_fb is None:
                self.capture()
            self.graph_fb.replay()
            if self.world > 1 and not self.ddp_graph:
                if self.overlap_comm:
                    w1 = w2 = None
                    if exchange and self.allpairs is not None:
                        main = torch.cuda.current_stream()
                        self._comm_stream.wait_stream(main)
                        with torch.cuda.stream(self._comm_stream):
                            self.allpairs(self.flat_g[self.bucket_off:])
                        self.graph_fb2.replay()
                        self.allpairs(self.flat_g[:self.bucket_off])
                        main.wait_stream(self._comm_stream)
                        self.graph_opt.replay()
                        self.steps_done += 1
                        return
                    if exchange:
                        w1 = dist.all_reduce(self.flat_g[self.bucket_off:], op=dist.ReduceOp.SUM, group=self.pg, async_op=True)
                    self.graph_fb2.replay()
                    if exchange:
                        w2 = dist.all_reduce(self.flat_g[:self.bucket_off], op=dist.ReduceOp.SUM, group=self.pg, async_op=True)
                        w1.wait(); w2.wait()
                elif exchange:
                    self._allreduce()
                self.graph_opt.replay()
        else:
            self._fwd_train(); self._loss(); self._backward()
            if exchange:
                self._allreduce()
            self._optimizer()
        self.steps_done += 1

    def forward_backward(self):
        self._fwd_train(); self._loss(tick=False); self._backward()

    def forward_only(self, images: torch.Tensor, labels: Optional[torch.Tensor] = None) -> torch.Tensor:
        if self.dataset is not None:
            raise L.VitpeError("a resident dataset is attached: use forward_indexed (or attach_dataset(None))")
        n = self._load_batch(images, labels)
        self._forward()
        return self.logits[:n]

    def kernel_probes(self):
        mdl, M, D, B, N, Hh, hid = self.model, self.M, self.D, self.B, self.N, self.H, self.hid
        G, es = self.Gr, 2 if self.T == torch.bfloat16 else 4
        hd = D // Hh
        probes = []
        attn_core_flop = 2 * 2 * N * N * hd * Hh * B
        qkv_flop = 2 * M * D * 3 * D
        attn_fwd = [(lambda l=l: self._attn_layer_fwd(l)) for l in range(self.Lyr)]
        attn_bwd = [(lambda l=l: self._attn_bwd(l, self.dx_mid[l])) for l in range(self.Lyr)]
        if self.attn_fused:
            probes.append(dict(name="attn_fwd", kernel=("attn32_fwd_kernel" if self.attn_wide else "attn_fwd_kernel") +
                               " (fused LN1+QKV-project+RoPE+QK^T+softmax+AV)",
                               fns=attn_fwd, flop=qkv_flop + attn_core_flop,
                               bytes=2 * M * D * es))
            if not self.fuse_ln:
                probes[-1]["kernel"] = probes[-1]["kernel"].replace("fused LN1+", "fused ")
            probes.append(dict(name="attn_bwd", kernel="attn_bwd_kernel (recompute + dQ/dK/dV + PE gradients -> d_qkv)",
                               fns=attn_bwd, flop=2 * (qkv_flop + attn_core_flop),
                               bytes=(2 + 3) * M * D * es))
        else:
            if self.attn_fused64:
                probes.append(dict(name="attn_fwd", kernel="attn_fused64_fwd_kernel (QKV-project+RoPE+QK^T+softmax+AV per (image, head), + raw qkv out)",
                                   fns=attn_fwd, flop=qkv_flop + attn_core_flop, bytes=(1 + 3 + 1) * M * D * es))
            else:
                probes.append(dict(name="attn_fwd", kernel="attn_core_fwd_kernel (RoPE+QK^T+softmax+AV per (image, head))",
                                   fns=attn_fwd, flop=attn_core_flop, bytes=4 * M * D * es))
            probes.append(dict(name="attn_bwd", kernel="attn_core_bwd_kernel", fns=attn_bwd, flop=2 * attn_core_flop,
                               bytes=(3 + 1 + 3) * M * D * es))
        if self.tail2 and self.group_wgrad:
            def tail_f(l):
                blk, a = mdl.blocks[l], self.act[l]
                nxt = (self.act[l + 1]["m1"], self.act[l + 1]["r1"]) if l + 1 < self.Lyr else None
                return lambda: self._block_tail_fwd(l, blk, a, nxt, save=True)
            def tail_b(l):
                blk, a = mdl.blocks[l], self.act[l]
                return lambda: self._block_tail_bwd(l, blk, a)
            tail_flop = 2 * M * D * D + 2 * 2 * M * D * hid
            probes.append(dict(name="block_tail_fwd",
                               kernel="block_tail2_fwd_kernel" +
                               " (proj+residual+LN2+fc1+GELU+fc2+residual+stats)",
                               fns=[tail_f(l) for l in range(self.Lyr)], flop=tail_flop,
                               bytes=self._tail_bytes(fwd=True)))
            probes.append(dict(name="block_tail_bwd",
                               kernel="block_tail2_bwd_kernel" +
                               " (gelu'+dgrad fc2/fc1+LN2 bwd+residual+dgrad proj)",
                               fns=[tail_b(l) for l in range(self.Lyr)], flop=tail_flop,
                               bytes=self._tail_bytes(fwd=False)))
            if self.fuse_lnbwd and self.Lyr > 1:
                def tail_bp(l):
                    blk, a = mdl.blocks[l], self.act[l]
                    return lambda: self._block_tail_bwd(l, blk, a, pre=True)
                probes.append(dict(name="block_tail_bwd_pre",
                                   kernel="block_tail2_bwd_kernel<PRE> (dgrad qkv + LN1 bwd of the block above, then the tail backward)",
                                   fns=[tail_bp(l) for l in range(self.Lyr - 1)], flop=tail_flop + 2 * M * D * 3 * D,
                                   bytes=self._tail_bytes(fwd=False) + (3 * M * D + 2 * M * D) * es))
            if self.lnbwd2:
                def dg(l):
                    blk, a = mdl.blocks[l], self.act[l]
                    return lambda: K.linear_lnbwd2(self.dqkv_l[l].view(M, 3 * D), self.Frt(blk.attn.qkv.weight),
                                                   self.x[l].view(M, D), a["m1"], a["r1"], blk.norm1.weight.data,
                                                   self.dx_mid[l].view(M, D), self.Gr(blk.norm1.weight), self.Gr(blk.norm1.bias),
                                                   out=self.dx_out[l].view(M, D))
                probes.append(dict(name="dgrad_qkv_ln1_bwd", kernel="ln_bwd2_kernel (dgrad qkv + LayerNorm1 backward + residual)",
                                   fns=[dg(l) for l in range(self.Lyr)], flop=2 * M * D * 3 * D,
                                   bytes=(3 * M * D + 3 * M * D) * es))
            self._wgrad_group("all") if "all" not in self._wg_groups else None
            wg_flop = sum(2 * dy.shape[0] * dy.shape[1] * x.shape[1] for grp in self._wg_groups["all"] for dy, x, _, _ in grp.keep)
            wg_bytes = sum((dy.numel() + x.numel()) * es + dw.numel() * 4 for grp in self._wg_groups["all"] for dy, x, dw, _ in grp.keep)
            probes.append(dict(name="wgrad_group", kernel="wgrad_group_kernel (every nn.Linear weight gradient, one launch)",
                               fns=[lambda: self._wgrad_group("all")], flop=wg_flop, bytes=wg_bytes))
        return probes

    def eval_loss(self, n: int, acc: torch.Tensor, n_global: Optional[int] = None):
        key = (n, n_global or n)
        if getattr(self, "_eval_ctl_key", None) != key:
            self._eval_ctl = torch.tensor([0.0, 1.0 / max(n_global or n, 1), float(n), 0.0], device=self.dev)
            self._eval_ctl_key = key
        ctl = self._eval_ctl
        K.cross_entropy_ctl(self.logits, self.labels, ctl, dlogits=None, out2=self.out2, metric_acc=acc)

    def read_metrics(self, reset=True):
        t = self.metric_acc
        if self.world > 1:
            t = self.metric_acc.clone()
            dist.all_reduce(t, op=dist.ReduceOp.SUM, group=self.pg)
        v = t.tolist()
        if reset:
            self.metric_acc.zero_()
        return v[0], v[1]
```

vit-rpe-rope_amd/vitpe/kernels.py:

```python
from __future__ import annotations

import ctypes
from typing import Optional, Tuple

import torch

from . import _lib as L
from ._lib import check, dtype_code, lib, ptr, require_device, stream_ptr

SPLITS_TARGET_WGS = 512


def _f32(t, name):
    if t is not None and t.dtype != torch.float32:
        raise L.VitpeError(f"{name} must be float32")


def gemm_nt(a, w, bias=None, epi=L.EPI_BIAS, resid=None, u=None, out=None):
    require_device(a, w, bias, resid, u, out)
    M, K = a.shape
    N = w.shape[0]
    assert w.shape[1] == K and a.dtype == w.dtype
    _f32(bias, "bias")
    c = out if out is not None else torch.empty((M, N), dtype=a.dtype, device=a.device)
    if epi == L.EPI_BIAS_GELU and u is None:
        u = torch.empty((M, N), dtype=a.dtype, device=a.device)
    check(lib().vitpe_gemm_nt(dtype_code(a.dtype), epi, ptr(a), ptr(w), ptr(c), ptr(bias), ptr(resid), ptr(u),
                              None, None, M, N, K, 0, 0, stream_ptr()), "vitpe_gemm_nt")
    return (c, u) if epi == L.EPI_BIAS_GELU else c


def linear(a, w, bias=None, epi=L.EPI_BIAS, resid=None, u=None, out=None, stats=None, eps=1e-5):
    require_device(a, w, bias, resid, u, out)
    M, K = a.shape
    N = w.shape[0]
    assert w.shape[1] == K and a.dtype == w.dtype
    _f32(bias, "bias")
    c = out if out is not None else torch.empty((M, N), dtype=a.dtype, device=a.device)
    if epi == L.EPI_BIAS_GELU and u is None:
        u = torch.empty((M, N), dtype=a.dtype, device=a.device)
    mean, rstd = stats if stats is not None else (None, None)
    require_device(mean, rstd)
    check(lib().vitpe_linear(dtype_code(a.dtype), epi, ptr(a), ptr(w), ptr(c), ptr(bias), ptr(resid), ptr(u),
                             ptr(mean), ptr(rstd), eps, M, N, K, stream_ptr()), "vitpe_linear")
    return (c, u) if epi == L.EPI_BIAS_GELU else c


def linear_ln(x, gamma, beta, mean, rstd, w, bias=None, epi=L.EPI_BIAS, u=None, out=None, xn_out=None):
    require_device(x, gamma, beta, mean, rstd, w, bias, u, out, xn_out)
    M, K = x.shape
    N = w.shape[0]
    c = out if out is not None else torch.empty((M, N), dtype=x.dtype, device=x.device)
    if epi == L.EPI_BIAS_GELU and u is None:
        u = torch.empty((M, N), dtype=x.dtype, device=x.device)
    check(lib().vitpe_linear_ln(dtype_code(x.dtype), epi, ptr(x), ptr(gamma), ptr(beta), ptr(mean), ptr(rstd),
                                ptr(xn_out), ptr(w), ptr(c), ptr(bias), ptr(u), M, N, K, stream_ptr()), "vitpe_linear_ln")
    return (c, u) if epi == L.EPI_BIAS_GELU else c


def linear_lnbwd(dy, wt, x, mean, rstd, gamma, dres, dgamma, dbeta, out=None):
    require_device(dy, wt, x, mean, rstd, gamma, dres, dgamma, dbeta, out)
    M, K = dy.shape
    assert wt.shape == (192, K) and x.shape[-1] == 192
    dx = out if out is not None else torch.empty((M, 192), dtype=dy.dtype, device=dy.device)
    check(lib().vitpe_linear_lnbwd(dtype_code(dy.dtype), ptr(dy), ptr(wt), ptr(dx), ptr(x), ptr(mean), ptr(rstd),
                                   ptr(gamma), ptr(dres), ptr(dgamma), ptr(dbeta), M, K, stream_ptr()),
          "vitpe_linear_lnbwd")
    return dx


def linear_lnbwd2(dy, wt_pk, x, mean, rstd, gamma, dres, dgamma, dbeta, out=None):
    require_device(dy, wt_pk, x, mean, rstd, gamma, dres, dgamma, dbeta, out)
    M, K = dy.shape
    assert wt_pk.numel() == 192 * K and x.shape[-1] == 192 and dy.dtype == wt_pk.dtype == x.dtype == dres.dtype
    _f32(gamma, "gamma"), _f32(dgamma, "dgamma"), _f32(dbeta, "dbeta"), _f32(mean, "mean"), _f32(rstd, "rstd")
    dx = out if out is not None else torch.empty((M, 192), dtype=dy.dtype, device=dy.device)
    check(lib().vitpe_linear_lnbwd2(dtype_code(dy.dtype), ptr(dy), ptr(wt_pk), ptr(dx), ptr(x), ptr(mean), ptr(rstd),
                                    ptr(gamma), ptr(dres), ptr(dgamma), ptr(dbeta), M, K, stream_ptr()),
          "vitpe_linear_lnbwd2")
    return dx


def patch_embed_gemm(patches, w, bias, cls, ape, B, P, out=None):
    require_device(patches, w, bias, cls, ape, out)
    M, K = patches.shape
    N = w.shape[0]
    assert M == B * P
    _f32(bias, "bias"), _f32(cls, "cls"), _f32(ape, "ape")
    c = out if out is not None else torch.empty((B, P + 1, N), dtype=patches.dtype, device=patches.device)
    check(lib().vitpe_gemm_nt(dtype_code(patches.dtype), L.EPI_PATCH, ptr(patches), ptr(w), ptr(c), ptr(bias), None,
                              None, ptr(ape), ptr(cls), M, N, K, P, P + 1, stream_ptr()), "vitpe_gemm_nt(patch)")
    return c


def wgrad_splits(M, N, K):
    tiles = ((N + 127) // 128) * ((K + 127) // 128 if (K % 128 == 0 or K > 192) else (K + 63) // 64)
    return max(1, min(64, SPLITS_TARGET_WGS // max(tiles, 1), (M + 255) // 256))


def gemm_tn(dy, x, dw, dbias=None, splits=None):
    require_device(dy, x, dw, dbias)
    M, N = dy.shape
    K = x.shape[1]
    assert x.shape[0] == M and dw.numel() == N * K and dy.dtype == x.dtype
    _f32(dw, "dw"), _f32(dbias, "dbias")
    if splits is None:
        splits = wgrad_splits(M, N, K)
    check(lib().vitpe_gemm_tn(dtype_code(dy.dtype), ptr(dy), ptr(x), ptr(dw), ptr(dbias), M, N, K, splits,
                              stream_ptr()), "vitpe_gemm_tn")


def pack_weight_frags(w, dtype, kchunk, phi, out=None):
    require_device(w, out)
    _f32(w, "w")
    R, C = w.shape
    out = out if out is not None else torch.empty((R, C), dtype=dtype, device=w.device)
    assert out.dtype == dtype and out.numel() == R * C
    check(lib().vitpe_pack_weight_frags(dtype_code(dtype), ptr(w), ptr(out), R, C, int(kchunk), int(bool(phi)), stream_ptr()),
          "vitpe_pack_weight_frags")
    return out


def block_tail2_supported(dtype, D, HID) -> bool:
    return bool(lib().vitpe_block_tail2_supported(dtype_code(dtype), int(D), int(HID)))


def block_tail2_fwd(attn_out, x_in, wp_pk, bp, gamma, beta, w1_pk, b1, w2_pk, b2, x_mid=None, mean2=None, rstd2=None,
                    xn_out=None, gp=None, h=None, out=None, stats=None, eps2=1e-5, eps_next=1e-5, save=True):
    require_device(attn_out, x_in, wp_pk, bp, gamma, beta, w1_pk, b1, w2_pk, b2, x_mid, mean2, rstd2, xn_out, gp, h, out)
    M, D = attn_out.shape
    HID = b1.numel()
    assert x_in.shape == (M, D) and wp_pk.numel() == D * D and w1_pk.numel() == HID * D and w2_pk.numel() == D * HID
    assert attn_out.dtype == x_in.dtype == wp_pk.dtype == w1_pk.dtype == w2_pk.dtype
    for t_, n_ in ((bp, "bp"), (gamma, "gamma"), (beta, "beta"), (b1, "b1"), (b2, "b2")):
        _f32(t_, n_)
    dt, dev = attn_out.dtype, attn_out.device
    x_mid = x_mid if x_mid is not None else torch.empty((M, D), dtype=dt, device=dev)
    mean2 = mean2 if mean2 is not None else torch.empty(M, dtype=torch.float32, device=dev)
    rstd2 = rstd2 if rstd2 is not None else torch.empty(M, dtype=torch.float32, device=dev)
    if save:
        gp = gp if gp is not None else torch.empty((M, HID), dtype=torch.float16, device=dev)
        h = h if h is not None else torch.empty((M, HID), dtype=dt, device=dev)
        assert gp.shape == h.shape == (M, HID) and h.dtype == dt and gp.dtype == torch.float16
    else:
        gp = h = None
    out = out if out is not None else torch.empty((M, D), dtype=dt, device=dev)
    mo, ro = stats if stats is not None else (None, None)
    require_device(mo, ro)
    check(lib().vitpe_block_tail2_fwd(dtype_code(dt), ptr(attn_out), ptr(x_in), ptr(wp_pk), ptr(bp), ptr(gamma), ptr(beta),
                                      ptr(x_mid), ptr(mean2), ptr(rstd2), ptr(xn_out), ptr(w1_pk), ptr(b1), ptr(w2_pk),
                                      ptr(b2), ptr(gp), ptr(h), ptr(out), ptr(mo), ptr(ro), float(eps2), float(eps_next),
                                      M, D, HID, stream_ptr()), "vitpe_block_tail2_fwd")
    return out, x_mid, mean2, rstd2, gp, h


def block_tail2_bwd(dy, gp, w2t_pk, w1t_pk, x_mid, mean2, rstd2, gamma, dgamma, dbeta, wpt_pk, du=None, out=None, da=None):
    require_device(dy, gp, w2t_pk, w1t_pk, x_mid, mean2, rstd2, gamma, dgamma, dbeta, wpt_pk, du, out, da)
    M, D = dy.shape
    HID = gp.shape[1]
    assert gp.shape == (M, HID) and x_mid.shape == (M, D) and w2t_pk.numel() == HID * D and w1t_pk.numel() == HID * D
    assert wpt_pk.numel() == D * D and dy.dtype == w2t_pk.dtype == w1t_pk.dtype == x_mid.dtype == wpt_pk.dtype
    assert gp.dtype == torch.float16
    _f32(gamma, "gamma"), _f32(dgamma, "dgamma"), _f32(dbeta, "dbeta"), _f32(mean2, "mean2"), _f32(rstd2, "rstd2")
    du = du if du is not None else torch.empty(gp.shape, dtype=dy.dtype, device=dy.device)
    out = out if out is not None else torch.empty_like(dy)
    da = da if da is not None else torch.empty_like(dy)
    check(lib().vitpe_block_tail2_bwd(dtype_code(dy.dtype), ptr(dy), ptr(gp), ptr(w2t_pk), ptr(w1t_pk), ptr(x_mid), ptr(mean2),
                                      ptr(rstd2), ptr(gamma), ptr(du), ptr(out), ptr(dgamma), ptr(dbeta), ptr(wpt_pk), ptr(da),
                                      M, D, HID, stream_ptr()), "vitpe_block_tail2_bwd")
    return out, du, da


def block_tail2_bwd_pre(dqkv, wqt_pk, x1, mean1, rstd1, gamma1, dres1, dgamma1, dbeta1, dy_out, gp, w2t_pk, w1t_pk, x_mid,
                        mean2, rstd2, gamma, dgamma, dbeta, wpt_pk, du=None, out=None, da=None):
    require_device(dqkv, wqt_pk, x1, mean1, rstd1, gamma1, dres1, dgamma1, dbeta1, dy_out, gp, w2t_pk, w1t_pk, x_mid, mean2,
                   rstd2, gamma, dgamma, dbeta, wpt_pk, du, out, da)
    M, K1 = dqkv.shape
    D, HID = dy_out.shape[1], gp.shape[1]
    assert dy_out.shape == (M, D) and gp.shape == (M, HID) and x_mid.shape == (M, D) and wqt_pk.numel() == D * K1
    assert dqkv.dtype == wqt_pk.dtype == dy_out.dtype == w2t_pk.dtype == w1t_pk.dtype == x_mid.dtype == wpt_pk.dtype
    assert gp.dtype == torch.float16
    for t_, n_ in ((gamma, "gamma"), (dgamma, "dgamma"), (dbeta, "dbeta"), (gamma1, "gamma1"), (dgamma1, "dgamma1"),
                   (dbeta1, "dbeta1"), (mean1, "mean1"), (rstd1, "rstd1"), (mean2, "mean2"), (rstd2, "rstd2")):
        _f32(t_, n_)
    du = du if du is not None else torch.empty(gp.shape, dtype=dy_out.dtype, device=dy_out.device)
    out = out if out is not None else torch.empty_like(dy_out)
    da = da if da is not None else torch.empty_like(dy_out)
    check(lib().vitpe_block_tail2_bwd_pre(dtype_code(dqkv.dtype), ptr(dqkv), ptr(wqt_pk), ptr(x1), ptr(mean1), ptr(rstd1),
                                          ptr(gamma1), ptr(dres1), ptr(dgamma1), ptr(dbeta1), K1, ptr(dy_out), ptr(gp),
                                          ptr(w2t_pk), ptr(w1t_pk), ptr(x_mid), ptr(mean2), ptr(rstd2), ptr(gamma), ptr(du),
                                          ptr(out), ptr(dgamma), ptr(dbeta), ptr(wpt_pk), ptr(da), M, D, HID, stream_ptr()),
          "vitpe_block_tail2_bwd_pre")
    return out, du, da


class _WgradProblem(ctypes.Structure):
    _fields_ = [("dY", ctypes.c_void_p), ("X", ctypes.c_void_p), ("dW", ctypes.c_void_p), ("dbias", ctypes.c_void_p),
                ("M", ctypes.c_int), ("N", ctypes.c_int), ("K", ctypes.c_int), ("x_op", ctypes.c_int),
                ("x_mean", ctypes.c_void_p), ("x_rstd", ctypes.c_void_p), ("x_gamma", ctypes.c_void_p),
                ("x_beta", ctypes.c_void_p)]


class WgradGroup:

    MAX = 28

    def __init__(self, problems):
        problems = [tuple(p) + (None,) * (5 - len(p)) for p in problems]
        if not 0 < len(problems) <= self.MAX:
            raise L.VitpeError(f"WgradGroup takes 1..{self.MAX} problems, got {len(problems)}")
        self.keep = [p[:4] for p in problems]
        self._ln = [p[4] for p in problems]
        self.dtype = problems[0][0].dtype
        self.arr = (_WgradProblem * len(problems))()
        for i, (dy, x, dw, db, ln) in enumerate(problems):
            require_device(dy, x, dw, db)
            M, N = dy.shape
            K = x.shape[1]
            assert x.shape[0] == M and dw.numel() == N * K and dy.dtype == x.dtype == self.dtype
            assert dy.is_contiguous() and x.is_contiguous() and dw.is_contiguous()
            _f32(dw, "dw"), _f32(db, "dbias")
            if ln is None:
                self.arr[i] = _WgradProblem(ptr(dy), ptr(x), ptr(dw), ptr(db), M, N, K, 0, None, None, None, None)
            else:
                mean, rstd, gamma, beta = ln
                require_device(mean, rstd, gamma, beta)
                for t_, n_ in ((mean, "mean"), (rstd, "rstd"), (gamma, "gamma"), (beta, "beta")):
                    _f32(t_, n_)
                assert mean.numel() == M and rstd.numel() == M and gamma.numel() == K and beta.numel() == K
                self.arr[i] = _WgradProblem(ptr(dy), ptr(x), ptr(dw), ptr(db), M, N, K, 1, ptr(mean), ptr(rstd), ptr(gamma),
                                            ptr(beta))

    def launch(self):
        check(lib().vitpe_wgrad_group(dtype_code(self.dtype), ctypes.addressof(self.arr), len(self.arr), stream_ptr()),
              "vitpe_wgrad_group")


def wgrad_group(problems):
    WgradGroup(problems).launch()


def layernorm_fwd(x, gamma, beta, eps=1e-5, out=None, mean=None, rstd=None, stats_only=False):
    require_device(x, gamma, beta, out)
    D = x.shape[-1]
    M = x.numel() // D
    _f32(gamma, "gamma"), _f32(beta, "beta")
    y = None if stats_only else (out if out is not None else torch.empty_like(x))
    mean = mean if mean is not None else torch.empty(M, dtype=torch.float32, device=x.device)
    rstd = rstd if rstd is not None else torch.empty(M, dtype=torch.float32, device=x.device)
    check(lib().vitpe_layernorm_fwd(dtype_code(x.dtype), ptr(x), ptr(gamma), ptr(beta), ptr(y), ptr(mean), ptr(rstd),
                                    M, D, eps, stream_ptr()), "vitpe_layernorm_fwd")
    return y, mean, rstd


def layernorm_bwd_workspace(M, D, device):
    return torch.empty(lib().vitpe_layernorm_bwd_blocks(M) * 2 * D, dtype=torch.float32, device=device)


def layernorm_bwd(dy, x, mean, rstd, gamma, dgamma, dbeta, dres=None, out=None, workspace=None):
    require_device(dy, x, mean, rstd, gamma, dgamma, dbeta, dres, out, workspace)
    D = x.shape[-1]
    M = x.numel() // D
    dx = out if out is not None else torch.empty_like(x)
    ws = workspace if workspace is not None else layernorm_bwd_workspace(M, D, x.device)
    check(lib().vitpe_layernorm_bwd(dtype_code(x.dtype), ptr(dy), ptr(x), ptr(mean), ptr(rstd), ptr(gamma), ptr(dres),
                                    ptr(dx), ptr(dgamma), ptr(dbeta), ptr(ws), M, D, stream_ptr()),
          "vitpe_layernorm_bwd")
    return dx


class PETables:

    def __init__(self, mode: str, grid: int, cos=None, sin=None, table=None, coeff=None, degree=0,
                 coeff_per_head=False):
        self.mode, self.grid = mode, grid
        self.cos, self.sin, self.table, self.coeff = cos, sin, table, coeff
        self.degree, self.coeff_per_head = degree, coeff_per_head

    @property
    def code(self):
        return L.PE_CODES[self.mode]


def _pe_tail(pe: PETables):
    return (pe.code, ptr(pe.cos), ptr(pe.sin), ptr(pe.table), ptr(pe.coeff), pe.grid, pe.degree, int(pe.coeff_per_head))


def _ln_variant(name, ln):
    if ln is None:
        return name, ()
    require_device(*ln)
    return name + "_ln", tuple(ptr(t) for t in ln)


def fused_attention_supported(dtype, N, D, HD) -> bool:
    return bool(lib().vitpe_fused_attention_supported(dtype_code(dtype), N, D, HD))


def pack_qkv_weights(wqkv_f32, dtype, num_heads, out=None):
    require_device(wqkv_f32, out)
    _f32(wqkv_f32, "wqkv")
    D = wqkv_f32.shape[1]
    o = out if out is not None else torch.empty((3 * D, D), dtype=dtype, device=wqkv_f32.device)
    check(lib().vitpe_pack_qkv_weights(dtype_code(dtype), ptr(wqkv_f32), ptr(o), D, D // num_heads, stream_ptr()),
          "vitpe_pack_qkv_weights")
    return o


def fused_attention_fwd(xn, wqkv, num_heads, pe: PETables, out=None, ln=None, xn_out=None):
    require_device(xn, wqkv, pe.cos, pe.sin, pe.table, pe.coeff, out, xn_out)
    B, N, D = xn.shape
    HD = D // num_heads
    assert wqkv.numel() == 3 * D * D and wqkv.dtype == xn.dtype
    o = out if out is not None else torch.empty_like(xn)
    name, lnp = _ln_variant("vitpe_fused_attention_fwd", ln)
    if ln is not None:
        lnp += (ptr(xn_out),)
    check(getattr(lib(), name)(dtype_code(xn.dtype), ptr(xn), *lnp, ptr(wqkv), ptr(o), B, N, D, HD, *_pe_tail(pe),
                               stream_ptr()), name)
    return o


def fused_attention_wide_supported(dtype, N, D, HD) -> bool:
    return bool(lib().vitpe_fused_attention_wide_supported(dtype_code(dtype), N, D, HD))


def pack_qkv_weights_wide(wqkv_f32, dtype, num_heads, out=None):
    require_device(wqkv_f32, out)
    _f32(wqkv_f32, "wqkv")
    D = wqkv_f32.shape[1]
    n = lib().vitpe_qkv_wide_pack_elems(D)
    o = out if out is not None else torch.empty(n, dtype=dtype, device=wqkv_f32.device)
    assert o.numel() == n and o.dtype == dtype
    check(lib().vitpe_pack_qkv_weights_wide(dtype_code(dtype), ptr(wqkv_f32), ptr(o), D, D // num_heads, stream_ptr()),
          "vitpe_pack_qkv_weights_wide")
    return o


def fused_attention_fwd_wide(xn, wqkv_wide, num_heads, pe: PETables, out=None, ln=None, xn_out=None):
    require_device(xn, wqkv_wide, pe.cos, pe.sin, pe.table, pe.coeff, out, xn_out)
    B, N, D = xn.shape
    HD = D // num_heads
    assert wqkv_wide.numel() == 3 * D * D and wqkv_wide.dtype == xn.dtype
    o = out if out is not None else torch.empty_like(xn)
    g = ln if ln is not None else (None, None, None, None)
    if ln is not None:
        require_device(*ln)
    check(lib().vitpe_fused_attention_fwd_wide(dtype_code(xn.dtype), ptr(xn), ptr(g[0]), ptr(g[1]), ptr(g[2]), ptr(g[3]),
                                               ptr(xn_out), ptr(wqkv_wide), ptr(o), B, N, D, HD, *_pe_tail(pe),
                                               stream_ptr()), "vitpe_fused_attention_fwd_wide")
    return o


def fused_attention_bwd(xn, wqkv, dout, num_heads, pe: PETables, dtable=None, dcoeff=None, dfreqs=None, out=None, ln=None):
    require_device(xn, wqkv, dout, dtable, dcoeff, dfreqs, out)
    B, N, D = xn.shape
    HD = D // num_heads
    dqkv = out if out is not None else torch.empty((B, N, 3 * D), dtype=xn.dtype, device=xn.device)
    name, lnp = _ln_variant("vitpe_fused_attention_bwd", ln)
    check(getattr(lib(), name)(dtype_code(xn.dtype), ptr(xn), *lnp, ptr(wqkv), ptr(dout), ptr(dqkv), B, N, D, HD,
                               *_pe_tail(pe), ptr(dtable), ptr(dcoeff), ptr(dfreqs), stream_ptr()), name)
    return dqkv


def attention_core_supported(dtype, N, HD):
    return bool(lib().vitpe_attention_core_supported(dtype_code(dtype), N, HD))


def attention_core_fwd(qkv, num_heads, pe: PETables, out=None):
    require_device(qkv, out)
    B, N, D3 = qkv.shape
    D = D3 // 3
    HD = D // num_heads
    o = out if out is not None else torch.empty((B, N, D), dtype=qkv.dtype, device=qkv.device)
    check(lib().vitpe_attention_core_fwd(dtype_code(qkv.dtype), ptr(qkv), ptr(o), B, N, num_heads, HD, *_pe_tail(pe),
                                         stream_ptr()), "vitpe_attention_core_fwd")
    return o


def attention_fused64_supported(dtype, N, num_heads, HD) -> bool:
    return bool(lib().vitpe_attention_fused64_supported(dtype_code(dtype), int(N), int(num_heads), int(HD)))


def attention_fused64_fwd(xn, wqkv_pk, num_heads, pe: PETables, qkv_out=None, out=None):
    require_device(xn, wqkv_pk, qkv_out, out, pe.cos, pe.sin, pe.table, pe.coeff)
    B, N, D = xn.shape
    HD = D // num_heads
    assert wqkv_pk.numel() == 3 * D * D and wqkv_pk.dtype == xn.dtype
    if qkv_out is not None:
        assert qkv_out.shape == (B, N, 3 * D) and qkv_out.dtype == xn.dtype and qkv_out.is_contiguous()
    o = out if out is not None else torch.empty_like(xn)
    check(lib().vitpe_attention_fused64_fwd(dtype_code(xn.dtype), ptr(xn), ptr(wqkv_pk), ptr(qkv_out), ptr(o), B, N, num_heads,
                                            HD, *_pe_tail(pe), stream_ptr()), "vitpe_attention_fused64_fwd")
    return o


def attention_core_bwd(qkv, dout, num_heads, pe: PETables, dtable=None, dcoeff=None, dfreqs=None, out=None,
                       dcos=None, dsin=None):
    require_device(qkv, dout, dtable, dcoeff, dfreqs, out, dcos, dsin)
    B, N, D3 = qkv.shape
    HD = D3 // 3 // num_heads
    dqkv = out if out is not None else torch.empty_like(qkv)
    if dcos is None and dsin is None:
        check(lib().vitpe_attention_core_bwd(dtype_code(qkv.dtype), ptr(qkv), ptr(dout), ptr(dqkv), B, N, num_heads, HD,
                                             *_pe_tail(pe), ptr(dtable), ptr(dcoeff), ptr(dfreqs),
                                             stream_ptr()), "vitpe_attention_core_bwd")
        return dqkv
    if dcos is None or dsin is None or pe.cos is None or dcos.shape != pe.cos.shape or dsin.shape != pe.sin.shape:
        raise L.VitpeError("attention_core_bwd: dcos and dsin must both be given, shaped like the rotary tables")
    _f32(dcos, "dcos"), _f32(dsin, "dsin")
    ws = torch.empty(4 * B * num_heads * (N - 1) * (HD // 2), dtype=torch.float32, device=qkv.device)
    check(lib().vitpe_attention_core_bwd_tables(dtype_code(qkv.dtype), ptr(qkv), ptr(dout), ptr(dqkv), B, N, num_heads, HD,
                                                *_pe_tail(pe), None, None, None, ptr(dcos), ptr(dsin), ptr(ws),
                                                stream_ptr()),
          "vitpe_attention_core_bwd_tables")
    return dqkv


SITE_ELEMENT, SITE_SAMPLE, SITE_ATTENTION = 0, 1, 2


def new_rng_pairs(n, device):
    return torch.empty((n, 2), dtype=torch.int64, device=device).random_()


def _check_rng(rng):
    require_device(rng)
    if rng.dtype != torch.int64 or rng.numel() != 2:
        raise L.VitpeError("rng must be a contiguous int64 device tensor of two words (seed, offset)")


def dropout_mask(rng, p, n=None, attn_shape=None):
    _check_rng(rng)
    if attn_shape is not None:
        B, H, N = attn_shape
        m = torch.empty((B, H, N, N), dtype=torch.uint8, device=rng.device)
        check(lib().vitpe_dropout_mask(SITE_ATTENTION, ptr(rng), ptr(m), 0, B, H, N, float(p), stream_ptr()),
              "vitpe_dropout_mask")
        return m
    m = torch.empty(n, dtype=torch.uint8, device=rng.device)
    check(lib().vitpe_dropout_mask(SITE_ELEMENT, ptr(rng), ptr(m), n, 0, 0, 0, float(p), stream_ptr()), "vitpe_dropout_mask")
    return m


def dropout_fwd(x, rng, p, resid=None, out=None):
    require_device(x, resid, out)
    _check_rng(rng)
    y = out if out is not None else torch.empty_like(x)
    assert resid is None or (resid.shape == x.shape and resid.dtype == x.dtype)
    check(lib().vitpe_dropout_fwd(dtype_code(x.dtype), ptr(x), ptr(resid), ptr(y), x.numel(), ptr(rng), float(p),
                                  stream_ptr()), "vitpe_dropout_fwd")
    return y


def dropout_bwd(dy, rng, p, out=None):
    require_device(dy, out)
    _check_rng(rng)
    dx = out if out is not None else torch.empty_like(dy)
    check(lib().vitpe_dropout_bwd(dtype_code(dy.dtype), ptr(dy), ptr(dx), dy.numel(), ptr(rng), float(p), stream_ptr()),
          "vitpe_dropout_bwd")
    return dx


def drop_path_fwd(x, rng, p, resid=None, out=None):
    require_device(x, resid, out)
    _check_rng(rng)
    y = out if out is not None else torch.empty_like(x)
    assert resid is None or (resid.shape == x.shape and resid.dtype == x.dtype)
    B = x.shape[0]
    check(lib().vitpe_drop_path_fwd(dtype_code(x.dtype), ptr(x), ptr(resid), ptr(y), B, x.numel() // max(B, 1), ptr(rng),
                                    float(p), stream_ptr()), "vitpe_drop_path_fwd")
    return y


def drop_path_bwd(dy, rng, p, out=None):
    require_device(dy, out)
    _check_rng(rng)
    dx = out if out is not None else torch.empty_like(dy)
    B = dy.shape[0]
    check(lib().vitpe_drop_path_bwd(dtype_code(dy.dtype), ptr(dy), ptr(dx), B, dy.numel() // max(B, 1), ptr(rng), float(p),
                                    stream_ptr()), "vitpe_drop_path_bwd")
    return dx


def attention_core_fwd_drop(qkv, num_heads, pe: PETables, rng, p, out=None):
    require_device(qkv, out)
    _check_rng(rng)
    B, N, D3 = qkv.shape
    D = D3 // 3
    HD = D // num_heads
    o = out if out is not None else torch.empty((B, N, D), dtype=qkv.dtype, device=qkv.device)
    check(lib().vitpe_attention_core_fwd_drop(dtype_code(qkv.dtype), ptr(qkv), ptr(o), B, N, num_heads, HD,
                                              *_pe_tail(pe), ptr(rng), float(p), stream_ptr()),
          "vitpe_attention_core_fwd_drop")
    return o


def attention_core_bwd_drop(qkv, dout, num_heads, pe: PETables, rng, p, dtable=None, dcoeff=None, dfreqs=None, out=None):
    require_device(qkv, dout, dtable, dcoeff, dfreqs, out)
    _check_rng(rng)
    B, N, D3 = qkv.shape
    HD = D3 // 3 // num_heads
    dqkv = out if out is not None else torch.empty_like(qkv)
    check(lib().vitpe_attention_core_bwd_drop(dtype_code(qkv.dtype), ptr(qkv), ptr(dout), ptr(dqkv), B, N, num_heads, HD,
                                              *_pe_tail(pe), ptr(dtable), ptr(dcoeff), ptr(dfreqs),
                                              ptr(rng), float(p), stream_ptr()), "vitpe_attention_core_bwd_drop")
    return dqkv


def unfold(images, patch, dtype, out=None):
    require_device(images, out)
    _f32(images, "images")
    B, C, S, _ = images.shape
    g = S // patch
    o = out if out is not None else torch.empty((B * g * g, C * patch * patch), dtype=dtype, device=images.device)
    check(lib().vitpe_unfold(dtype_code(dtype), ptr(images), ptr(o), B, C, S, patch, stream_ptr()), "vitpe_unfold")
    return o


def unfold_u8(data, index, mean, std, patch, dtype, out=None, img_out=None):
    require_device(data, index, mean, std, out, img_out)
    if data.dtype != torch.uint8 or (index is not None and index.dtype != torch.int64):
        raise L.VitpeError("unfold_u8: data must be uint8 and index int64")
    _f32(mean, "mean"), _f32(std, "std"), _f32(img_out, "img_out")
    _, C, S, _ = data.shape
    B = index.shape[0] if index is not None else data.shape[0]
    g = S // patch
    o = out if out is not None else torch.empty((B * g * g, C * patch * patch), dtype=dtype, device=data.device)
    check(lib().vitpe_unfold_u8(dtype_code(dtype), ptr(data), ptr(index), ptr(mean), ptr(std), ptr(o), ptr(img_out), B, C, S,
                                patch, stream_ptr()), "vitpe_unfold_u8")
    return o


def resize_coeffs(size_in: int, size_out: int):
    size_in, size_out = int(size_in), int(size_out)
    if size_in < 1 or size_out < 1:
        raise L.VitpeError(f"resize_coeffs: sizes must be positive (got {size_in} -> {size_out})")
    ksize = 2 * -(-max(size_in, size_out) // size_out) + 1
    bounds = torch.zeros((size_out, 2), dtype=torch.int32)
    kk = torch.zeros((size_out, ksize), dtype=torch.int32)
    got = lib().vitpe_resize_coeffs(size_in, size_out, bounds.data_ptr(), kk.data_ptr(), ksize)
    if got != ksize:
        raise L.VitpeError(f"vitpe_resize_coeffs({size_in}, {size_out}) returned {got}, expected ksize {ksize}")
    return bounds, kk


def resize_u8_supported(S0: int, S: int) -> bool:
    return bool(lib().vitpe_resize_u8_supported(int(S0), int(S)))


def resize_u8(images_u8, S: int, out=None):
    require_device(images_u8, out)
    S = int(S)
    if images_u8.dtype != torch.uint8 or images_u8.dim() != 4 or images_u8.shape[2] != images_u8.shape[3]:
        raise L.VitpeError("resize_u8: images must be uint8 [N,C,S0,S0] (square)")
    N, C, S0, _ = images_u8.shape
    if not resize_u8_supported(S0, S):
        raise L.VitpeError(f"resize_u8: {S0} -> {S} is not supported (source 8..64, target 4..512)")
    if out is None:
        out = torch.empty((N, C, S, S), dtype=torch.uint8, device=images_u8.device)
    elif out.dtype != torch.uint8 or out.numel() < N * C * S * S:
        raise L.VitpeError("resize_u8: out must be uint8 with at least N*C*S*S elements")
    bounds = kk = None
    ksize = 0
    if S != S0:
        bounds, kk = (t.to(images_u8.device) for t in resize_coeffs(S0, S))
        ksize = kk.shape[1]
    check(lib().vitpe_resize_u8(ptr(images_u8), ptr(out), N * C, S0, S, ptr(bounds), ptr(kk), ptr(bounds), ptr(kk), ksize,
                                stream_ptr()), "vitpe_resize_u8")
    return out


def patch_embed_supported(dtype, C, S, p, D) -> bool:
    return bool(lib().vitpe_patch_embed_supported(dtype_code(dtype), C, S, p, D))


def patch_embed(w, bias, cls, ape, patch, dtype, images=None, data=None, index=None, mean=None, std=None, out=None,
                patches_out=None, stats=None, eps=1e-5):
    require_device(w, bias, cls, ape, images, data, index, mean, std, out, patches_out)
    src = images if images is not None else data
    C, S = src.shape[1], src.shape[2]
    B = images.shape[0] if images is not None else (index.shape[0] if index is not None else data.shape[0])
    D = w.shape[0]
    P = (S // patch) ** 2
    assert w.dtype == dtype and w.shape[1] == C * patch * patch
    _f32(bias, "bias"), _f32(cls, "cls"), _f32(ape, "ape"), _f32(images, "images")
    o = out if out is not None else torch.empty((B, P + 1, D), dtype=dtype, device=w.device)
    mo, ro = stats if stats is not None else (None, None)
    require_device(mo, ro)
    check(lib().vitpe_patch_embed(dtype_code(dtype), ptr(images), ptr(data), ptr(index), ptr(mean), ptr(std), ptr(w), ptr(bias),
                                  ptr(cls), ptr(ape), ptr(o), ptr(patches_out), ptr(mo), ptr(ro), B, C, S, patch, D, float(eps),
                                  stream_ptr()), "vitpe_patch_embed")
    return o


def embed_bwd(dtok, dcls, dape, out=None):
    require_device(dtok, dcls, dape, out)
    B, Ntok, D = dtok.shape
    dpatch = out if out is not None else torch.empty((B * (Ntok - 1), D), dtype=dtok.dtype, device=dtok.device)
    check(lib().vitpe_embed_bwd(dtype_code(dtok.dtype), ptr(dtok), ptr(dcls), ptr(dape), ptr(dpatch), B, Ntok, D,
                                stream_ptr()), "vitpe_embed_bwd")
    return dpatch


def relative_position_index(L_, device):
    out = torch.empty((L_, L_), dtype=torch.int64, device=device)
    require_device(out)
    check(lib().vitpe_relative_position_index(ptr(out), L_, stream_ptr()), "vitpe_relative_position_index")
    return out


def l1_distance_matrix(G, device):
    out = torch.empty((G * G, G * G), dtype=torch.int64, device=device)
    require_device(out)
    check(lib().vitpe_l1_distance_matrix(ptr(out), G, stream_ptr()), "vitpe_l1_distance_matrix")
    return out


def rope_axial_tables(inv_freq, grid):
    require_device(inv_freq)
    half = inv_freq.numel() * 2
    cos = torch.empty((grid * grid, half), dtype=torch.float32, device=inv_freq.device)
    sin = torch.empty_like(cos)
    check(lib().vitpe_rope_axial_tables(ptr(inv_freq), ptr(cos), ptr(sin), grid, half, stream_ptr()),
          "vitpe_rope_axial_tables")
    return cos, sin


def rope_mixed_tables(freqs, grid, cos=None, sin=None):
    require_device(freqs, cos, sin)
    _, H, half = freqs.shape
    if cos is None:
        cos = torch.empty((H, grid * grid, half), dtype=torch.float32, device=freqs.device)
        sin = torch.empty_like(cos)
    check(lib().vitpe_rope_mixed_tables(ptr(freqs), ptr(cos), ptr(sin), H, grid, half, stream_ptr()),
          "vitpe_rope_mixed_tables")
    return cos, sin


def relative_bias(table, L_):
    require_device(table)
    H = table.shape[0]
    out = torch.empty((H, L_, L_), dtype=torch.float32, device=table.device)
    check(lib().vitpe_relative_bias(ptr(table), ptr(out), H, L_, stream_ptr()), "vitpe_relative_bias")
    return out


def polynomial_bias(coeff, H, grid, degree, per_head):
    require_device(coeff)
    L_ = grid * grid + 1
    out = torch.empty((H, L_, L_), dtype=torch.float32, device=coeff.device)
    check(lib().vitpe_polynomial_bias(ptr(coeff), ptr(out), H, grid, degree, int(per_head), stream_ptr()),
          "vitpe_polynomial_bias")
    return out


def relative_bias_bwd(dbias, L_):
    require_device(dbias)
    _f32(dbias, "dbias")
    H = dbias.shape[0]
    out = torch.empty((H, 2 * L_ - 1), dtype=torch.float32, device=dbias.device)
    check(lib().vitpe_relative_bias_bwd(ptr(dbias), ptr(out), H, L_, stream_ptr()), "vitpe_relative_bias_bwd")
    return out


def polynomial_bias_bwd(dbias, H, grid, degree, per_head):
    require_device(dbias)
    _f32(dbias, "dbias")
    out = torch.empty((H, degree + 1) if per_head else (degree + 1,), dtype=torch.float32, device=dbias.device)
    check(lib().vitpe_polynomial_bias_bwd(ptr(dbias), ptr(out), H, grid, degree, int(per_head), stream_ptr()),
          "vitpe_polynomial_bias_bwd")
    return out


def rope_mixed_tables_bwd(freqs, dcos, dsin, grid):
    require_device(freqs, dcos, dsin)
    _f32(dcos, "dcos"), _f32(dsin, "dsin")
    _, H, half = freqs.shape
    out = torch.empty_like(freqs)
    check(lib().vitpe_rope_mixed_tables_bwd(ptr(freqs), ptr(dcos), ptr(dsin), ptr(out), H, grid, half, stream_ptr()),
          "vitpe_rope_mixed_tables_bwd")
    return out


def apply_rotary(x, cos, sin):
    require_device(x, cos, sin)
    _f32(x, "x")
    B, H, P, HD = x.shape
    per_head = cos.dim() == 3
    y = torch.empty_like(x)
    check(lib().vitpe_apply_rotary(ptr(x), ptr(y), ptr(cos), ptr(sin), B, H, P, HD, int(per_head), stream_ptr()),
          "vitpe_apply_rotary")
    return y


def apply_rotary_bwd(dy, x, cos, sin, dcos=None, dsin=None, want_dx=True):
    require_device(dy, x, cos, sin, dcos, dsin)
    _f32(dy, "dy"), _f32(x, "x"), _f32(dcos, "dcos"), _f32(dsin, "dsin")
    B, H, P, HD = dy.shape
    per_head = cos.dim() == 3
    for t in (dcos, dsin):
        if t is not None and t.shape != cos.shape:
            raise L.VitpeError("apply_rotary_bwd: dcos / dsin must be shaped like cos / sin")
    dx = torch.empty_like(dy) if want_dx else None
    ws = None
    if dcos is not None or dsin is not None:
        R = B if per_head else B * H
        ws = torch.empty(2 * min(R, 64) * (H if per_head else 1) * P * (HD // 2), dtype=torch.float32, device=dy.device)
    check(lib().vitpe_apply_rotary_bwd(ptr(dy), ptr(x), ptr(cos), ptr(sin), ptr(dx), ptr(dcos), ptr(dsin), ptr(ws), B, H, P,
                                       HD, int(per_head), stream_ptr()), "vitpe_apply_rotary_bwd")
    return dx


def head_fwd(x, gamma, beta, wh, bh, eps=1e-5, save=False, logits=None, ws=None):
    require_device(x, gamma, beta, wh, bh, logits)
    B, Ntok, D = x.shape
    Cn = wh.shape[0]
    lg = logits if logits is not None else torch.empty((B, Cn), dtype=torch.float32, device=x.device)
    if save and ws is None:
        ws = (torch.empty((B, D), dtype=torch.float32, device=x.device),
              torch.empty((B, D), dtype=torch.float32, device=x.device),
              torch.empty((B,), dtype=torch.float32, device=x.device))
    w0, w1, w2 = ws if ws is not None else (None, None, None)
    check(lib().vitpe_head_fwd(dtype_code(x.dtype), ptr(x), ptr(gamma), ptr(beta), ptr(wh), ptr(bh), ptr(lg), ptr(w0),
                               ptr(w1), ptr(w2), B, Ntok, D, Cn, eps, stream_ptr()), "vitpe_head_fwd")
    return lg, ws


def cross_entropy(logits, labels, grad_scale=None, dlogits=None, out2=None, want_grad=True):
    require_device(logits, labels, dlogits, out2)
    B, Cn = logits.shape
    assert labels.dtype == torch.int64
    if want_grad and dlogits is None:
        dlogits = torch.empty_like(logits)
    o = out2 if out2 is not None else torch.empty(2, dtype=torch.float32, device=logits.device)
    gs = (1.0 / B) if grad_scale is None else grad_scale
    check(lib().vitpe_cross_entropy(ptr(logits), ptr(labels), ptr(dlogits), ptr(o), B, Cn, gs, stream_ptr()),
          "vitpe_cross_entropy")
    return o, dlogits


def cross_entropy_ctl(logits, labels, ctl, dlogits=None, out2=None, metric_acc=None):
    require_device(logits, labels, ctl, dlogits, out2, metric_acc)
    B, Cn = logits.shape
    assert labels.dtype == torch.int64 and ctl.dtype == torch.float32 and ctl.numel() >= 3
    _f32(dlogits, "dlogits"), _f32(out2, "out2"), _f32(metric_acc, "metric_acc")
    o = out2 if out2 is not None else torch.empty(2, dtype=torch.float32, device=logits.device)
    check(lib().vitpe_cross_entropy_ctl(ptr(logits), ptr(labels), ptr(dlogits), ptr(o), ptr(metric_acc), ptr(ctl), B, Cn,
                                        stream_ptr()), "vitpe_cross_entropy_ctl")
    return o, dlogits


def head_bwd(dlogits, wh, gamma, ws, dtype, Ntok, dwh, dbh, dgamma, dbeta, dx=None, ws_dyn=None):
    require_device(dlogits, wh, gamma, dwh, dbh, dgamma, dbeta, dx, ws_dyn)
    B, Cn = dlogits.shape
    D = wh.shape[1]
    if dx is None:
        dx = torch.empty((B, Ntok, D), dtype=dtype, device=dlogits.device)
    if ws_dyn is None:
        ws_dyn = torch.empty((B, D), dtype=torch.float32, device=dlogits.device)
    check(lib().vitpe_head_bwd(dtype_code(dtype), ptr(dlogits), ptr(wh), ptr(gamma), ptr(ws[0]), ptr(ws[1]),
                               ptr(ws[2]), ptr(ws_dyn), ptr(dx), ptr(dwh), ptr(dbh), ptr(dgamma), ptr(dbeta), B, Ntok,
                               D, Cn, stream_ptr()), "vitpe_head_bwd")
    return dx


def head_loss(x, gamma, beta, wh, bh, labels, logits, dlogits, ws, ws_dyn, dx, out2, metric_acc, scratch, dwh, dbh,
              dgamma, dbeta, eps=1e-5, grad_scale=None):
    require_device(x, gamma, beta, wh, bh, labels, logits, dlogits, ws[0], ws[1], ws_dyn, dx, out2, metric_acc, scratch, dwh,
                   dbh, dgamma, dbeta)
    B, Ntok, D = x.shape
    Cn = wh.shape[0]
    assert labels.dtype == torch.int64 and scratch.numel() >= 4
    gs = (1.0 / B) if grad_scale is None else grad_scale
    check(lib().vitpe_head_loss(dtype_code(x.dtype), ptr(x), ptr(gamma), ptr(beta), ptr(wh), ptr(bh), ptr(labels), ptr(logits),
                                ptr(dlogits), ptr(ws[0]), ptr(ws[1]), ptr(ws_dyn), ptr(dx), ptr(out2), ptr(metric_acc),
                                ptr(scratch), ptr(dwh), ptr(dbh), ptr(dgamma), ptr(dbeta), B, Ntok, D, Cn, float(eps),
                                float(gs), stream_ptr()), "vitpe_head_loss")


def head_step(x, gamma, beta, wh, bh, labels, logits, dlogits, ws, ws_dyn, dx, out2, metric_acc, per_image, ctl, dwh, dbh,
              dgamma, dbeta, eps=1e-5, hp_tick=None):
    require_device(x, gamma, beta, wh, bh, labels, logits, dlogits, ws[0], ws[1], ws_dyn, dx, out2, metric_acc, per_image, ctl,
                   dwh, dbh, dgamma, dbeta, hp_tick)
    B, Ntok, D = x.shape
    Cn = wh.shape[0]
    assert labels.dtype == torch.int64 and per_image.numel() >= 2 * B and ctl.numel() >= 3
    check(lib().vitpe_head_step(dtype_code(x.dtype), ptr(x), ptr(gamma), ptr(beta), ptr(wh), ptr(bh), ptr(labels), ptr(logits),
                                ptr(dlogits), ptr(ws[0]), ptr(ws[1]), ptr(ws_dyn), ptr(dx), ptr(out2), ptr(metric_acc),
                                ptr(per_image), ptr(ctl), ptr(dwh), ptr(dbh), ptr(dgamma), ptr(dbeta), B, Ntok, D, Cn, float(eps),
                                ptr(hp_tick), stream_ptr()), "vitpe_head_step")


def adamw_step(p, g, m, v, hp, shadow_bf16=None, zero_grad=True, ticked=False):
    require_device(p, g, m, v, hp, shadow_bf16)
    check(lib().vitpe_adamw_step(ptr(p), ptr(g), ptr(m), ptr(v), ptr(shadow_bf16), ptr(hp), p.numel(),
                                 int(bool(zero_grad)) | (2 if ticked else 0),
                                 stream_ptr()), "vitpe_adamw_step")


def cast(src, dtype, out=None):
    require_device(src, out)
    _f32(src, "src")
    o = out if out is not None else torch.empty(src.shape, dtype=dtype, device=src.device)
    check(lib().vitpe_cast(dtype_code(dtype), ptr(src), ptr(o), src.numel(), stream_ptr()), "vitpe_cast")
    return o


def transpose_cast(src, dtype, out=None):
    require_device(src, out)
    _f32(src, "src")
    R, C = src.shape
    o = out if out is not None else torch.empty((C, R), dtype=dtype, device=src.device)
    check(lib().vitpe_transpose_cast(dtype_code(dtype), ptr(src), ptr(o), R, C, stream_ptr()), "vitpe_transpose_cast")
    return o


def refresh_shadows(flat, dst_base, desc, ndesc, total_tiles, tile_map=None):
    require_device(flat, dst_base, desc, tile_map)
    assert tile_map is None or (tile_map.dtype == torch.int16 and tile_map.numel() == total_tiles)
    check(lib().vitpe_refresh_shadows(dtype_code(dst_base.dtype), ptr(flat), ptr(dst_base), ptr(desc), ndesc, total_tiles,
                                      ptr(tile_map), stream_ptr()), "vitpe_refresh_shadows")


def selftest_mma(a, bt, brow):
    require_device(a, bt, brow)
    c_row = torch.empty((16, 16), dtype=torch.float32, device=a.device)
    c_tr = torch.empty((16, 16), dtype=torch.float32, device=a.device)
    check(L.debug_lib().vitpe_selftest_mma(dtype_code(a.dtype), ptr(a), ptr(bt), ptr(brow), ptr(c_row), ptr(c_tr),
                                   stream_ptr()), "vitpe_selftest_mma")
    return c_row, c_tr
```

Baseline: 337,200 images/sec.

## Compute last block's MLP tail only for CLS rows with strided weight-grad

Adds fused forward and backward kernels that run the last block's projection, LayerNorm, MLP and residual only on the CLS-token rows (one row per image, selected by a row stride). The strided rows also feed a row-subsampled weight-gradient group path, and small problems get extra short work slots. Since only the CLS token reaches the classifier, this skips tail work on every other token of the top layer. It adds new kernels, scheduling complexity and separate scratch buffers.

```diff
diff --git a/include/vitpe.h b/include/vitpe.h
--- a/include/vitpe.h
+++ b/include/vitpe.h
@@ -129,6 +129,14 @@
                               const void* x_mid, const float* mean2, const float* rstd2, const float* gamma, void* du,
                               void* dx_mid, float* dgamma, float* dbeta, const void* WpT_packed, void* da, int M, int D,
                               int HID, vitpe_stream_t stream);
+int vitpe_tail_cls_fwd(int dtype, const void* attn_out, const void* x_in, const void* Wp_packed, const float* bp,
+                       const float* gamma, const float* beta, void* x_mid, float* mean2, float* rstd2, void* xn_out,
+                       const void* W1_packed, const float* b1, const void* W2_packed, const float* b2, void* gp_out,
+                       void* h_out, void* out, float eps2, int B, int row_step, int D, int HID, vitpe_stream_t stream);
+int vitpe_tail_cls_bwd(int dtype, const void* dy, const void* gp, const void* W2t_packed, const void* W1t_packed,
+                       const void* x_mid, const float* mean2, const float* rstd2, const float* gamma, void* du,
+                       void* dx_mid, float* dgamma, float* dbeta, const void* WpT_packed, void* da, int B, int row_step,
+                       int D, int HID, vitpe_stream_t stream);
 int vitpe_gemm_tn(int dtype, const void* dY, const void* X, float* dW, float* dbias, int M, int N,
                   int K, int splits, vitpe_stream_t stream);
 
@@ -147,6 +155,8 @@
 #define VITPE_XOP_NONE 0
 #define VITPE_XOP_LAYERNORM 1
 int vitpe_wgrad_group(int dtype, const vitpe_wgrad_problem* problems, int nprob, vitpe_stream_t stream);
+int vitpe_wgrad_group_rows(int dtype, const vitpe_wgrad_problem* problems, const int* row_step, int nprob,
+                           vitpe_stream_t stream);
 
 int vitpe_layernorm_fwd(int dtype, const void* x, const float* gamma, const float* beta, void* y,
                         float* mean, float* rstd, int M, int D, float eps, vitpe_stream_t stream);
diff --git a/vit-rpe-rope_amd/csrc/tail_cls.hip b/vit-rpe-rope_amd/csrc/tail_cls.hip
--- /dev/null
+++ b/vit-rpe-rope_amd/csrc/tail_cls.hip
@@ -0,0 +1,294 @@
+#include "common.h"
+
+namespace vitpe {
+
+constexpr int TC_D = 192, TC_NT = 12, TC_KS = 6, TC_THREADS = 64 * TC_NT, TC_MAXHID = 1536;
+constexpr int TC_XLD = TC_D + 8;
+constexpr int TC_FLD = TC_D + 4;
+constexpr int TC_HPAD = 8;
+
+struct TailClsFwdArgs {
+  const bf16* a;  const bf16* xin;
+  const bf16* wp; const float* bp; const float* gamma; const float* beta;
+  const bf16* w1; const float* b1; const bf16* w2; const float* b2;
+  bf16* xmid; float* mean2; float* rstd2;
+  bf16* xn_out;
+  _Float16* gp_out;
+  bf16* h_out;
+  bf16* out;
+  int B, HID, row_step;
+  float eps2;
+};
+
+VITPE_DEV void tc_st4(bf16* p, const f32x4& v) { st4(p, v[0], v[1], v[2], v[3]); }
+
+VITPE_DEV Frag<bf16> tc_phi_frag(const bf16* chunk_plus_4g) {
+  const bf16x4 lo = *reinterpret_cast<const bf16x4*>(chunk_plus_4g), hi = *reinterpret_cast<const bf16x4*>(chunk_plus_4g + 16);
+  Frag<bf16> f;
+  f.v = __builtin_shufflevector(lo, hi, 0, 1, 2, 3, 4, 5, 6, 7);
+  return f;
+}
+
+VITPE_DEV void tc_gelu(float x, float& h, float& g) {
+  constexpr float C = 0.39894228040143267794f;
+  const float ax = fabsf(x);
+  const float T = __builtin_amdgcn_rcpf(fmaf(ax, 0.3275911f * 0.70710678118654752440f, 1.0f));
+  float q = fmaf(T, 1.061405429f / (2.f * C), -1.453152027f / (2.f * C));
+  q = fmaf(T, q, 1.421413741f / (2.f * C));
+  q = fmaf(T, q, -0.284496736f / (2.f * C));
+  q = fmaf(T, q, 0.254829592f / (2.f * C));
+  const float E = __builtin_amdgcn_exp2f(fmaf(x * x, -0.72134752044448170368f, -1.32574806473615827f));
+  const float H = (q * T) * E;
+  h = fmaf(-ax, H, fmaxf(x, 0.f));
+  const float r = fmaf(ax, E, -H);
+  g = x >= 0.f ? 1.0f + r : -r;
+}
+
+__global__ __launch_bounds__(TC_THREADS) void tail_cls_fwd_kernel(TailClsFwdArgs a) {
+  constexpr int D = TC_D, NT = TC_NT, KS = TC_KS;
+  __shared__ __attribute__((aligned(16))) bf16 sX[16 * TC_XLD];
+  __shared__ __attribute__((aligned(16))) bf16 sH[16 * (TC_MAXHID + TC_HPAD)];
+  const int lane = threadIdx.x & 63, c = lane & 15, g = lane >> 4;
+  const int wave = __builtin_amdgcn_readfirstlane(threadIdx.x >> 6);
+  const int HID = a.HID, HLD = HID + TC_HPAD;
+  const size_t row = (size_t)min(16 * (int)blockIdx.x + c, a.B - 1) * a.row_step;
+  const int f0 = 16 * wave + 4 * g;
+
+  f32x4 xm_own;
+  {
+    const bf16* ar = a.a + row * D + 8 * g;
+    const bf16* wf = a.wp + (size_t)wave * KS * 512 + lane * 8;
+    Frag<bf16> fa[KS], fw[KS];
+#pragma unroll
+    for (int ks = 0; ks < KS; ++ks) { fw[ks] = ld_frag(wf + ks * 512); fa[ks] = ld_frag(ar + 32 * ks); }
+    const bf16x4 xr = *reinterpret_cast<const bf16x4*>(a.xin + row * D + f0);
+    f32x4 acc = *reinterpret_cast<const f32x4*>(a.bp + f0);
+#pragma unroll
+    for (int ks = 0; ks < KS; ++ks) mma(fw[ks], fa[ks], acc);
+#pragma unroll
+    for (int r = 0; r < 4; ++r) acc[r] = to_f32(from_f32<bf16>(acc[r] + (float)xr[r]));
+    xm_own = acc;
+    tc_st4(a.xmid + row * D + f0, acc);
+    tc_st4(sX + c * TC_XLD + f0, acc);
+  }
+  __syncthreads();
+
+  Frag<bf16> bf[KS];
+  {
+    f32x4 xa[NT];
+    float s1 = 0.f;
+#pragma unroll
+    for (int nt = 0; nt < NT; ++nt) {
+      xa[nt] = ld4(sX + c * TC_XLD + 16 * nt + 4 * g);
+#pragma unroll
+      for (int r = 0; r < 4; ++r) s1 += xa[nt][r];
+    }
+    const float invD = 1.0f / (float)D;
+    const float mean = xgroup_sum(s1) * invD;
+    float s2 = 0.f;
+#pragma unroll
+    for (int nt = 0; nt < NT; ++nt)
+#pragma unroll
+      for (int r = 0; r < 4; ++r) { const float d = xa[nt][r] - mean; s2 += d * d; }
+    const float rstd = 1.0f / sqrtf(xgroup_sum(s2) * invD + a.eps2);
+    if (wave == 0 && g == 0) { a.mean2[row] = mean; a.rstd2[row] = rstd; }
+#pragma unroll
+    for (int nt = 0; nt < NT; ++nt) {
+      const f32x4 gv = *reinterpret_cast<const f32x4*>(a.gamma + 16 * nt + 4 * g);
+      const f32x4 bv = *reinterpret_cast<const f32x4*>(a.beta + 16 * nt + 4 * g);
+#pragma unroll
+      for (int r = 0; r < 4; ++r) xa[nt][r] = fmaf((xa[nt][r] - mean) * rstd, gv[r], bv[r]);
+    }
+#pragma unroll
+    for (int ks = 0; ks < KS; ++ks) {
+      bf[ks] = acc_to_frag<bf16>(xa[2 * ks], xa[2 * ks + 1]);
+      if (a.xn_out != nullptr && ks == wave) {
+        bf16* xr = a.xn_out + row * D + 32 * ks + 4 * g;
+        *reinterpret_cast<bf16x4*>(xr) = __builtin_shufflevector(bf[ks].v, bf[ks].v, 0, 1, 2, 3);
+        *reinterpret_cast<bf16x4*>(xr + 16) = __builtin_shufflevector(bf[ks].v, bf[ks].v, 4, 5, 6, 7);
+      }
+    }
+  }
+
+  const bool save = a.gp_out != nullptr;
+  for (int nt = wave; nt < HID / 16; nt += NT) {
+    const bf16* wf = a.w1 + (size_t)nt * KS * 512 + lane * 8;
+    Frag<bf16> fw[KS];
+#pragma unroll
+    for (int ks = 0; ks < KS; ++ks) fw[ks] = ld_frag(wf + ks * 512);
+    f32x4 acc = *reinterpret_cast<const f32x4*>(a.b1 + 16 * nt + 4 * g);
+#pragma unroll
+    for (int ks = 0; ks < KS; ++ks) mma(fw[ks], bf[ks], acc);
+    f32x4 hh, gp;
+#pragma unroll
+    for (int r = 0; r < 4; ++r) { float hv, gv; tc_gelu(acc[r], hv, gv); hh[r] = hv; gp[r] = gv; }
+    tc_st4(sH + c * HLD + 16 * nt + 4 * g, hh);
+    if (save) {
+      tc_st4(a.h_out + row * HID + 16 * nt + 4 * g, hh);
+      const uint2 pk = {__builtin_bit_cast(uint32_t, __builtin_amdgcn_cvt_pkrtz(gp[0], gp[1])),
+                        __builtin_bit_cast(uint32_t, __builtin_amdgcn_cvt_pkrtz(gp[2], gp[3]))};
+      *reinterpret_cast<uint2*>(a.gp_out + row * HID + 16 * nt + 4 * g) = pk;
+    }
+  }
+  __syncthreads();
+
+  {
+    f32x4 acc = *reinterpret_cast<const f32x4*>(a.b2 + f0);
+    const bf16* wf = a.w2 + (size_t)wave * 512 + lane * 8;
+    const bf16* hr = sH + c * HLD + 4 * g;
+    for (int kc = 0; kc < HID / 32; ++kc) mma(ld_frag(wf + (size_t)kc * NT * 512), tc_phi_frag(hr + 32 * kc), acc);
+#pragma unroll
+    for (int r = 0; r < 4; ++r) acc[r] += xm_own[r];
+    tc_st4(a.out + row * D + f0, acc);
+  }
+}
+
+struct TailClsBwdArgs {
+  const bf16* dy; const _Float16* gp; const bf16* xmid; const float* mean2; const float* rstd2; const float* gamma;
+  const bf16* w2t; const bf16* w1t; const bf16* wpt;
+  bf16* du; bf16* dxmid; bf16* da;
+  float* dgamma; float* dbeta;
+  int B, HID, row_step;
+};
+
+__global__ __launch_bounds__(TC_THREADS) void tail_cls_bwd_kernel(TailClsBwdArgs a) {
+  constexpr int D = TC_D, NT = TC_NT, KS = TC_KS;
+  __shared__ __attribute__((aligned(16))) float sDx[16 * TC_FLD];
+  __shared__ __attribute__((aligned(16))) bf16 sDu[16 * (TC_MAXHID + TC_HPAD)];
+  const int lane = threadIdx.x & 63, c = lane & 15, g = lane >> 4;
+  const int wave = __builtin_amdgcn_readfirstlane(threadIdx.x >> 6);
+  const int HID = a.HID, HLD = HID + TC_HPAD;
+  const int lrow = 16 * (int)blockIdx.x + c;
+  const size_t row = (size_t)min(lrow, a.B - 1) * a.row_step;
+  const float valid = lrow < a.B ? 1.0f : 0.0f;
+  const int f0 = 16 * wave + 4 * g;
+
+  const bf16* const dyr = a.dy + row * D + 4 * g;
+  Frag<bf16> bf[KS];
+#pragma unroll
+  for (int ks = 0; ks < KS; ++ks) bf[ks] = tc_phi_frag(dyr + 32 * ks);
+  for (int nt = wave; nt < HID / 16; nt += NT) {
+    const bf16* wf = a.w2t + (size_t)nt * KS * 512 + lane * 8;
+    Frag<bf16> fw[KS];
+#pragma unroll
+    for (int ks = 0; ks < KS; ++ks) fw[ks] = ld_frag(wf + ks * 512);
+    const uint2 gw = *reinterpret_cast<const uint2*>(a.gp + row * HID + 16 * nt + 4 * g);
+    f32x4 acc = {0.f, 0.f, 0.f, 0.f};
+#pragma unroll
+    for (int ks = 0; ks < KS; ++ks) mma(fw[ks], bf[ks], acc);
+    f32x4 d;
+    d[0] = acc[0] * (float)__builtin_bit_cast(_Float16, (unsigned short)(gw.x & 0xffffu));
+    d[1] = acc[1] * (float)__builtin_bit_cast(_Float16, (unsigned short)(gw.x >> 16));
+    d[2] = acc[2] * (float)__builtin_bit_cast(_Float16, (unsigned short)(gw.y & 0xffffu));
+    d[3] = acc[3] * (float)__builtin_bit_cast(_Float16, (unsigned short)(gw.y >> 16));
+    tc_st4(a.du + row * HID + 16 * nt + 4 * g, d);
+    tc_st4(sDu + c * HLD + 16 * nt + 4 * g, d);
+  }
+  __syncthreads();
+
+  {
+    f32x4 acc = {0.f, 0.f, 0.f, 0.f};
+    const bf16* wf = a.w1t + (size_t)wave * 512 + lane * 8;
+    const bf16* dr = sDu + c * HLD + 4 * g;
+    for (int kc = 0; kc < HID / 32; ++kc) mma(ld_frag(wf + (size_t)kc * NT * 512), tc_phi_frag(dr + 32 * kc), acc);
+    *reinterpret_cast<f32x4*>(sDx + c * TC_FLD + f0) = acc;
+  }
+  __syncthreads();
+
+  f32x4 acc[NT];
+  {
+    const float mean = a.mean2[row], rstd = a.rstd2[row];
+    const bf16* xr = a.xmid + row * D + 4 * g;
+    const float invD = 1.0f / (float)D;
+    bf16x4 xmv[NT];
+    float s1 = 0.f, s2 = 0.f;
+#pragma unroll
+    for (int nt = 0; nt < NT; ++nt) {
+      xmv[nt] = *reinterpret_cast<const bf16x4*>(xr + 16 * nt);
+      acc[nt] = *reinterpret_cast<const f32x4*>(sDx + c * TC_FLD + 16 * nt + 4 * g);
+      const f32x4 gam = *reinterpret_cast<const f32x4*>(a.gamma + 16 * nt + 4 * g);
+      float tg[4], tb[4];
+#pragma unroll
+      for (int r = 0; r < 4; ++r) {
+        const float xhat = ((float)xmv[nt][r] - mean) * rstd;
+        const float dxn = acc[nt][r];
+        tg[r] = dxn * xhat * valid;
+        tb[r] = dxn * valid;
+        const float gy = dxn * gam[r];
+        s1 += gy;
+        s2 = fmaf(gy, xhat, s2);
+      }
+      if (nt == wave) {
+#pragma unroll
+        for (int r = 0; r < 4; ++r) {
+          const float sg = group16_sum(tg[r]), sb = group16_sum(tb[r]);
+          if (c == 0) { atomicAdd(a.dgamma + 16 * nt + 4 * g + r, sg); atomicAdd(a.dbeta + 16 * nt + 4 * g + r, sb); }
+        }
+      }
+    }
+    const float m1 = xgroup_sum(s1) * invD, m2 = xgroup_sum(s2) * invD;
+#pragma unroll
+    for (int nt = 0; nt < NT; ++nt) {
+      const bf16x4 rv = *reinterpret_cast<const bf16x4*>(dyr + 16 * nt);
+      const f32x4 gam = *reinterpret_cast<const f32x4*>(a.gamma + 16 * nt + 4 * g);
+#pragma unroll
+      for (int r = 0; r < 4; ++r) {
+        const float xhat = ((float)xmv[nt][r] - mean) * rstd;
+        const float gy = acc[nt][r] * gam[r];
+        acc[nt][r] = to_f32(from_f32<bf16>(fmaf(rstd, gy - m1 - xhat * m2, (float)rv[r])));
+      }
+      if (nt == wave) tc_st4(a.dxmid + row * D + 16 * nt + 4 * g, acc[nt]);
+    }
+  }
+
+  {
+    const bf16* wf = a.wpt + (size_t)wave * KS * 512 + lane * 8;
+    Frag<bf16> fwp[KS];
+#pragma unroll
+    for (int ks = 0; ks < KS; ++ks) fwp[ks] = ld_frag(wf + ks * 512);
+    f32x4 o = {0.f, 0.f, 0.f, 0.f};
+#pragma unroll
+    for (int ks = 0; ks < KS; ++ks) mma(fwp[ks], acc_to_frag<bf16>(acc[2 * ks], acc[2 * ks + 1]), o);
+    tc_st4(a.da + row * D + f0, o);
+  }
+}
+
+}
+
+using namespace vitpe;
+
+extern "C" int vitpe_block_tail2_supported(int dtype, int D, int HID);
+
+extern "C" int vitpe_tail_cls_fwd(int dtype, const void* attn_out, const void* x_in, const void* Wp_packed, const float* bp,
+                                  const float* gamma, const float* beta, void* x_mid, float* mean2, float* rstd2, void* xn_out,
+                                  const void* W1_packed, const float* b1, const void* W2_packed, const float* b2, void* gp_out,
+                                  void* h_out, void* out, float eps2, int B, int row_step, int D, int HID, hipStream_t stream) {
+  VITPE_REQUIRE(attn_out && x_in && Wp_packed && bp && gamma && beta && x_mid && mean2 && rstd2 && W1_packed && b1 &&
+                W2_packed && b2 && out && B >= 0 && row_step >= 1);
+  VITPE_REQUIRE((gp_out == nullptr) == (h_out == nullptr));
+  if (!vitpe_block_tail2_supported(dtype, D, HID)) return (int)hipErrorNotSupported;
+  if (B == 0) return 0;
+  TailClsFwdArgs a{};
+  a.a = (const bf16*)attn_out; a.xin = (const bf16*)x_in; a.wp = (const bf16*)Wp_packed; a.bp = bp; a.gamma = gamma; a.beta = beta;
+  a.w1 = (const bf16*)W1_packed; a.b1 = b1; a.w2 = (const bf16*)W2_packed; a.b2 = b2; a.xmid = (bf16*)x_mid; a.mean2 = mean2;
+  a.rstd2 = rstd2; a.xn_out = (bf16*)xn_out; a.gp_out = (_Float16*)gp_out; a.h_out = (bf16*)h_out; a.out = (bf16*)out;
+  a.B = B; a.HID = HID; a.row_step = row_step; a.eps2 = eps2;
+  hipLaunchKernelGGL(tail_cls_fwd_kernel, dim3((B + 15) / 16), dim3(TC_THREADS), 0, stream, a);
+  VITPE_CHECK_LAUNCH();
+}
+
+extern "C" int vitpe_tail_cls_bwd(int dtype, const void* dy, const void* gp, const void* W2t_packed, const void* W1t_packed,
+                                  const void* x_mid, const float* mean2, const float* rstd2, const float* gamma, void* du,
+                                  void* dx_mid, float* dgamma, float* dbeta, const void* WpT_packed, void* da, int B, int row_step,
+                                  int D, int HID, hipStream_t stream) {
+  VITPE_REQUIRE(dy && gp && W2t_packed && W1t_packed && x_mid && mean2 && rstd2 && gamma && du && dx_mid && dgamma && dbeta &&
+                WpT_packed && da && B >= 0 && row_step >= 1);
+  if (!vitpe_block_tail2_supported(dtype, D, HID)) return (int)hipErrorNotSupported;
+  if (B == 0) return 0;
+  TailClsBwdArgs a{};
+  a.dy = (const bf16*)dy; a.gp = (const _Float16*)gp; a.xmid = (const bf16*)x_mid; a.mean2 = mean2; a.rstd2 = rstd2; a.gamma = gamma;
+  a.w2t = (const bf16*)W2t_packed; a.w1t = (const bf16*)W1t_packed; a.wpt = (const bf16*)WpT_packed; a.du = (bf16*)du;
+  a.dxmid = (bf16*)dx_mid; a.da = (bf16*)da; a.dgamma = dgamma; a.dbeta = dbeta; a.B = B; a.HID = HID; a.row_step = row_step;
+  hipLaunchKernelGGL(tail_cls_bwd_kernel, dim3((B + 15) / 16), dim3(TC_THREADS), 0, stream, a);
+  VITPE_CHECK_LAUNCH();
+}
diff --git a/vit-rpe-rope_amd/csrc/wgrad.hip b/vit-rpe-rope_amd/csrc/wgrad.hip
--- a/vit-rpe-rope_amd/csrc/wgrad.hip
+++ b/vit-rpe-rope_amd/csrc/wgrad.hip
@@ -17,6 +17,7 @@
   const float* xbeta;
   int M, N, K;
   int xop;
+  int rs;
   int unit0;
   int nbn;
   int stages;
@@ -29,6 +30,8 @@
   int full_rounds, total_blocks;
   int tail_rounds;
   int bk;
+  int nbig;
+  int short_slots;
   int range_major;
   unsigned long long* census;
   WgProb p[WG_MAXPROB];
@@ -36,6 +39,7 @@
 };
 static_assert(sizeof(WgArgs) <= 4096, "kernel argument block");
 constexpr int WG_CENSUS_STAGES = 24, WG_CENSUS_SLOTS = 4;
+constexpr int WG_SHORT_SPR = 2;
 
 template <typename T> struct WgLayout;
 template <> struct WgLayout<bf16> {
@@ -71,7 +75,26 @@
 };
 
 template <class RunFn>
+VITPE_DEV void wg_dispatch_placed(const WgArgs& a, RunFn run);
+
+template <class RunFn>
 VITPE_DEV void wg_dispatch(const WgArgs& a, RunFn run) {
+  wg_dispatch_placed(a, run);
+  for (int s = blockIdx.x; s < a.short_slots; s += gridDim.x) {
+    int q = s, pi = a.nbig;
+    for (int i = a.nbig; i < a.nprob - 1; ++i) {
+      const int nsl = a.p[i].nbn * ((a.p[i].K + a.bk - 1) / a.bk) * ((a.p[i].stages + WG_SHORT_SPR - 1) / WG_SHORT_SPR);
+      if (pi == i && q >= nsl) { q -= nsl; pi = i + 1; }
+    }
+    const WgProb& P = a.p[pi];
+    const int nr = (P.stages + WG_SHORT_SPR - 1) / WG_SHORT_SPR;
+    const int ub = P.unit0 + (q / nr) * P.stages, u0 = ub + (q % nr) * WG_SHORT_SPR;
+    run(u0, min(ub + P.stages, u0 + WG_SHORT_SPR));
+  }
+}
+
+template <class RunFn>
+VITPE_DEV void wg_dispatch_placed(const WgArgs& a, RunFn run) {
   if (a.use_table == 2) {
     const int G = gridDim.x, idx = (blockIdx.x & 7) * (G >> 3) + (blockIdx.x >> 3);
     const int nrounds = a.range_major ? a.full_rounds : a.full_rounds + a.tail_rounds;
@@ -93,7 +116,7 @@
       }
       if (gb >= a.total_blocks) continue;
       int pi = 0, b0 = 0;
-      for (int i = 0; i < a.nprob; ++i) {
+      for (int i = 0; i < a.nbig; ++i) {
         const int nb = a.p[i].nbn * ((a.p[i].K + a.bk - 1) / a.bk);
         if (gb >= b0 + nb) { b0 += nb; pi = i + 1; } else break;
       }
@@ -140,7 +163,7 @@
   struct Cur {
     const T* dY; const T* X; float* dW; float* dbias;
     const float* xmean; const float* xrstd; const float* xgamma; const float* xbeta;
-    int M, N, K, n0, k0, stage, stages, xop;
+    int M, N, K, n0, k0, stage, stages, xop, rs;
   };
   auto decode = [&](int u, Cur& s) {
     int pi = 0;
@@ -151,7 +174,7 @@
     s.M = P.M; s.N = P.N; s.K = P.K; s.stages = P.stages;
     s.xmean = P.xop ? P.xmean : reinterpret_cast<const float*>(P.dY);
     s.xrstd = P.xop ? P.xrstd : reinterpret_cast<const float*>(P.dY);
-    s.xgamma = P.xgamma; s.xbeta = P.xbeta; s.xop = P.xop;
+    s.xgamma = P.xgamma; s.xbeta = P.xbeta; s.xop = P.xop; s.rs = P.rs;
     s.stage = ub - blk * P.stages;
     s.n0 = (blk % P.nbn) * WG_BLK;
     s.k0 = (blk / P.nbn) * a.bk;
@@ -170,13 +193,13 @@
       const int gm = mb + row;
       if (i < 2) {
         const int gn = s.n0 + cc * CHN;
-        rg[i] = (gm < s.M && gn < s.N) ? *reinterpret_cast<const Chunk16*>(s.dY + (size_t)gm * s.N + gn) : zero;
+        rg[i] = (gm < s.M && gn < s.N) ? *reinterpret_cast<const Chunk16*>(s.dY + (size_t)gm * s.rs * s.N + gn) : zero;
       } else {
         const int gk = s.k0 + cc * CHN;
         const bool ok = gm < s.M && gk < s.K;
-        rg[i] = ok ? *reinterpret_cast<const Chunk16*>(s.X + (size_t)gm * s.K + gk) : zero;
+        rg[i] = ok ? *reinterpret_cast<const Chunk16*>(s.X + (size_t)gm * s.rs * s.K + gk) : zero;
         if (LNX) {
-          const int gs = (s.xop == 1) ? min(gm, s.M - 1) : 0;
+          const size_t gs = (s.xop == 1) ? (size_t)min(gm, s.M - 1) * s.rs : 0;
           lnA[i - 2] = s.xrstd[gs];
           lnB[i - 2] = s.xmean[gs];
         }
@@ -472,21 +495,27 @@
   return n;
 }
 
-static int wgrad_group_launch(int dtype, const void* problems, int nprob, unsigned long long* census, hipStream_t stream);
+static int wgrad_group_launch(int dtype, const void* problems, const int* row_step, int nprob, unsigned long long* census,
+                              hipStream_t stream);
 static bool g_wide_ok = true;
 extern "C" int vitpe_debug_set_wgrad_wide(int on) { g_wide_ok = on != 0; return 0; }
 
 extern "C" int vitpe_wgrad_group(int dtype, const void* problems, int nprob, hipStream_t stream) {
-  return wgrad_group_launch(dtype, problems, nprob, nullptr, stream);
+  return wgrad_group_launch(dtype, problems, nullptr, nprob, nullptr, stream);
+}
+
+extern "C" int vitpe_wgrad_group_rows(int dtype, const void* problems, const int* row_step, int nprob, hipStream_t stream) {
+  return wgrad_group_launch(dtype, problems, row_step, nprob, nullptr, stream);
 }
 
 extern "C" int vitpe_debug_wgrad_census(int dtype, const void* problems, int nprob, unsigned long long* census,
                                         hipStream_t stream) {
   VITPE_REQUIRE(census != nullptr && dtype == 1);
-  return wgrad_group_launch(dtype, problems, nprob, census, stream);
-}
-
-static int wgrad_group_launch(int dtype, const void* problems, int nprob, unsigned long long* census, hipStream_t stream) {
+  return wgrad_group_launch(dtype, problems, nullptr, nprob, census, stream);
+}
+
+static int wgrad_group_launch(int dtype, const void* problems, const int* row_step, int nprob, unsigned long long* census,
+                              hipStream_t stream) {
   VITPE_REQUIRE(problems && nprob >= 0 && nprob <= WG_MAXPROB && (dtype == 0 || dtype == 1));
   const vitpe_wgrad_problem_abi* pr = reinterpret_cast<const vitpe_wgrad_problem_abi*>(problems);
   const int RPS = dtype == 1 ? 64 : 32, CHN = dtype == 1 ? 8 : 4;
@@ -494,27 +523,40 @@
   a.census = census;
   bool wide = g_wide_ok && dtype == 1 && census == nullptr && nprob > 0;
   for (int i = 0; i < nprob; ++i)
-    wide = wide && (pr[i].M == 0 || (pr[i].x_op == 0 && pr[i].N % WG_BLK == 0 && pr[i].K % WW_BK == 0));
+    wide = wide && (pr[i].M == 0 || (pr[i].x_op == 0 && pr[i].N % WG_BLK == 0 && pr[i].K % WW_BK == 0 &&
+                                     (row_step == nullptr || row_step[i] <= 1)));
   a.bk = wide ? WW_BK : WG_BLK;
-  int units = 0, np = 0;
-  for (int i = 0; i < nprob; ++i) {
-    const vitpe_wgrad_problem_abi& p = pr[i];
-    VITPE_REQUIRE(p.dY && p.X && p.dW && p.M >= 0 && p.N > 0 && p.K > 0 && p.N % CHN == 0 && p.K % CHN == 0);
-    if (p.M == 0) continue;
-    WgProb& q = a.p[np++];
-    VITPE_REQUIRE(p.x_op == 0 || (p.x_op == 1 && p.x_mean && p.x_rstd && p.x_gamma && p.x_beta));
-    q.dY = p.dY; q.X = p.X; q.dW = p.dW; q.dbias = p.dbias; q.M = p.M; q.N = p.N; q.K = p.K;
-    q.xop = p.x_op; q.xmean = p.x_mean; q.xrstd = p.x_rstd; q.xgamma = p.x_gamma; q.xbeta = p.x_beta;
-    q.unit0 = units;
-    q.nbn = (p.N + WG_BLK - 1) / WG_BLK;
-    q.stages = (p.M + RPS - 1) / RPS;
-    const long long nu = (long long)q.nbn * ((p.K + a.bk - 1) / a.bk) * q.stages;
-    VITPE_REQUIRE(units + nu < (1LL << 30));
-    units += (int)nu;
+  int max_stages = 0;
+  for (int i = 0; i < nprob; ++i) max_stages = (pr[i].M + RPS - 1) / RPS > max_stages ? (pr[i].M + RPS - 1) / RPS : max_stages;
+  int units = 0, np = 0, nbig = 0;
+  for (int pass = 0; pass < 2; ++pass) {
+    for (int i = 0; i < nprob; ++i) {
+      const vitpe_wgrad_problem_abi& p = pr[i];
+      VITPE_REQUIRE(p.dY && p.X && p.dW && p.M >= 0 && p.N > 0 && p.K > 0 && p.N % CHN == 0 && p.K % CHN == 0);
+      VITPE_REQUIRE(row_step == nullptr || row_step[i] >= 1);
+      if (p.M == 0) continue;
+      const int stages = (p.M + RPS - 1) / RPS;
+      if ((stages * 8 <= max_stages) != (pass == 1)) continue;
+      WgProb& q = a.p[np++];
+      VITPE_REQUIRE(p.x_op == 0 || (p.x_op == 1 && p.x_mean && p.x_rstd && p.x_gamma && p.x_beta));
+      q.dY = p.dY; q.X = p.X; q.dW = p.dW; q.dbias = p.dbias; q.M = p.M; q.N = p.N; q.K = p.K;
+      q.xop = p.x_op; q.xmean = p.x_mean; q.xrstd = p.x_rstd; q.xgamma = p.x_gamma; q.xbeta = p.x_beta;
+      q.rs = row_step != nullptr ? row_step[i] : 1;
+      q.unit0 = units;
+      q.nbn = (p.N + WG_BLK - 1) / WG_BLK;
+      q.stages = stages;
+      const long long nu = (long long)q.nbn * ((p.K + a.bk - 1) / a.bk) * q.stages;
+      VITPE_REQUIRE(units + nu < (1LL << 30));
+      units += (int)nu;
+    }
+    if (pass == 0) nbig = np;
   }
   if (units == 0) return 0;
   a.nprob = np;
+  a.nbig = nbig;
   a.total_units = units;
+  const int np_all = np;
+  np = nbig;
   const int ncu = wgrad_cu_count();
   int grid = 0;
   int total_blocks = 0, max_blocks = 0, min_stages = 1 << 30;
@@ -588,6 +630,11 @@
       (void)bestk;
     }
   }
+  if (a.use_table) {
+    for (int i = nbig; i < np_all; ++i)
+      a.short_slots += a.p[i].nbn * ((a.p[i].K + a.bk - 1) / a.bk) * ((a.p[i].stages + WG_SHORT_SPR - 1) / WG_SHORT_SPR);
+  }
+  np = np_all;
   if (!a.use_table) {
     const int wgs = units < ncu ? units : ncu;
     a.units_per_wg = (units + wgs - 1) / wgs;
diff --git a/vit-rpe-rope_amd/vitpe/engine.py b/vit-rpe-rope_amd/vitpe/engine.py
--- a/vit-rpe-rope_amd/vitpe/engine.py
+++ b/vit-rpe-rope_amd/vitpe/engine.py
@@ -268,6 +268,9 @@
         self.head_scratch = torch.zeros(2 * B, dtype=torch.float32, device=dev)
         self.fuse_head = self.Cn <= 64 and self.D <= 768 and os.environ.get("VITPE_FUSE_HEAD", "1") == "1"
         self.head_ws = (f(B, D), f(B, D), f(B))
+        self.cls_rows = (self.tail2 and self.group_wgrad and self.fuse_head and T == torch.bfloat16 and self.Lyr >= 2
+                         and os.environ.get("VITPE_CLS_ROWS", "1") == "1")
+        self._probe_scratch = None
         self.ws_dyn = f(B, D)
         self.dtmp = e(B, N, D)
         self.dx_out = [e(B, N, D) for _ in range(self.Lyr + 1)]
@@ -277,6 +280,14 @@
         self.dqkv_l = [e(B, N, 3 * D) for _ in range(self.Lyr)]
         self.qkv_l = [] if self.attn_fused else [e(B, N, 3 * D) for _ in range(self.Lyr)]
         self.dqkv, self.du = self.dqkv_l[0], self.du_l[0]
+        self.da_top = None
+        if self.cls_rows:
+            self.da_top = torch.zeros(B, N, D, dtype=T, device=dev)
+            top = self.act[self.Lyr - 1]
+            for t in (self.du_l[self.Lyr - 1], self.dx_mid[self.Lyr - 1], self.x[self.Lyr], top["xmid"], top["m2"], top["r2"],
+                      top["u"], top["h"], top["xn2"]):
+                if t is not None:
+                    t.zero_()
         self.dataset, self.batch_idx = None, None
         self._wg_groups = {}
         self.dpatch = e(B * self.P, D)
@@ -358,21 +369,45 @@
             K.head_fwd(self.x[-1], mdl.norm.weight.data, mdl.norm.bias.data, mdl.head.weight.data, mdl.head.bias.data,
                        mdl.norm.eps, save=True, logits=self.logits, ws=self.head_ws)
 
-    def _block_tail_fwd(self, l, blk, a, nxt, save=None):
+    def _top_cls(self, l):
+        return self.cls_rows and l == self.Lyr - 1
+
+    def _block_tail_fwd(self, l, blk, a, nxt, save=None, scratch=None):
         M, D = self.M, self.D
         eps_next = self.model.blocks[min(l + 1, self.Lyr - 1)].norm1.eps
         if save is None:
             save = self._save_hidden
+        if self._top_cls(l) and scratch is None:
+            K.tail_cls_fwd(a["a"].view(M, D), self.x[l].view(M, D), self.Fr(blk.attn.proj.weight), blk.attn.proj.bias.data,
+                           blk.norm2.weight.data, blk.norm2.bias.data, self.Fr(blk.mlp.fc1.weight), blk.mlp.fc1.bias.data,
+                           self.Fr(blk.mlp.fc2.weight), blk.mlp.fc2.bias.data, self.B, self.N, a["xmid"].view(M, D), a["m2"],
+                           a["r2"], self.x[l + 1].view(M, D),
+                           xn_out=(a["xn2"].view(M, D) if (save and not self.recompute_ln) else None),
+                           gp=(a["u"].view(torch.float16) if save else None), h=(a["h"] if save else None), eps2=blk.norm2.eps)
+            return
+        o = scratch if scratch is not None else dict(a, xout=self.x[l + 1])
         K.block_tail2_fwd(a["a"].view(M, D), self.x[l].view(M, D), self.Fr(blk.attn.proj.weight),
                           blk.attn.proj.bias.data, blk.norm2.weight.data, blk.norm2.bias.data,
                           self.Fr(blk.mlp.fc1.weight), blk.mlp.fc1.bias.data, self.Fr(blk.mlp.fc2.weight),
-                          blk.mlp.fc2.bias.data, x_mid=a["xmid"].view(M, D), mean2=a["m2"], rstd2=a["r2"],
-                          xn_out=(a["xn2"].view(M, D) if (save and not self.recompute_ln) else None),
-                          gp=(a["u"].view(torch.float16) if save else None), h=(a["h"] if save else None), out=self.x[l + 1].view(M, D),
+                          blk.mlp.fc2.bias.data, x_mid=o["xmid"].view(M, D), mean2=o["m2"], rstd2=o["r2"],
+                          xn_out=(o["xn2"].view(M, D) if (save and not self.recompute_ln) else None),
+                          gp=(o["u"].view(torch.float16) if save else None), h=(o["h"] if save else None), out=o["xout"].view(M, D),
                           stats=nxt, eps2=blk.norm2.eps, eps_next=eps_next, save=save)
 
-    def _block_tail_bwd(self, l, blk, a, pre=False):
+    def _block_tail_bwd(self, l, blk, a, pre=False, scratch=None):
         M, D, G = self.M, self.D, self.Gr
+        if self._top_cls(l) and scratch is None:
+            K.tail_cls_bwd(self.dx_out[l + 1].view(M, D), a["u"].view(torch.float16), self.Frt(blk.mlp.fc2.weight),
+                           self.Frt(blk.mlp.fc1.weight), a["xmid"].view(M, D), a["m2"], a["r2"], blk.norm2.weight.data,
+                           G(blk.norm2.weight), G(blk.norm2.bias), self.Frt(blk.attn.proj.weight), self.B, self.N,
+                           du=self.du_l[l], out=self.dx_mid[l].view(M, D), da=self.da_top.view(M, D))
+            return
+        if scratch is not None:
+            K.block_tail2_bwd(self.dx_out[l + 1].view(M, D), scratch["u"].view(torch.float16), self.Frt(blk.mlp.fc2.weight),
+                              self.Frt(blk.mlp.fc1.weight), scratch["xmid"].view(M, D), scratch["m2"], scratch["r2"],
+                              blk.norm2.weight.data, G(blk.norm2.weight), G(blk.norm2.bias), self.Frt(blk.attn.proj.weight),
+                              du=scratch["du"], out=scratch["dxmid"].view(M, D), da=self.dtmp.view(M, D))
+            return
         if pre:
             up, ua = self.model.blocks[l + 1], self.act[l + 1]
             K.block_tail2_bwd_pre(self.dqkv_l[l + 1].view(M, 3 * D), self.Frt(up.attn.qkv.weight), self.x[l + 1].view(M, D),
@@ -421,8 +456,11 @@
             else:
                 fc1 = (self.du_l[l], a["xn2"].view(M, D), G(blk.mlp.fc1.weight), G(blk.mlp.fc1.bias))
                 qkv = (self.dqkv_l[l].view(M, 3 * D), a["xn1"].view(M, D), G(blk.attn.qkv.weight), None)
-            probs += [(self.dx_out[l + 1].view(M, D), a["h"], G(blk.mlp.fc2.weight), G(blk.mlp.fc2.bias)), fc1,
-                      (self.dx_mid[l].view(M, D), a["a"].view(M, D), G(blk.attn.proj.weight), G(blk.attn.proj.bias)), qkv]
+            fc2 = (self.dx_out[l + 1].view(M, D), a["h"], G(blk.mlp.fc2.weight), G(blk.mlp.fc2.bias))
+            proj = (self.dx_mid[l].view(M, D), a["a"].view(M, D), G(blk.attn.proj.weight), G(blk.attn.proj.bias))
+            if self._top_cls(l):
+                fc2, fc1, proj = ((p + (None,) * (5 - len(p)) + (self.N,)) for p in (fc2, fc1, proj))
+            probs += [fc2, fc1, proj, qkv]
         if with_embed:
             probs.append((self.dpatch, self.patches, G(mdl.patch_embed.weight).view(D, -1), G(mdl.patch_embed.bias)))
         return probs
@@ -484,7 +522,7 @@
             self._wgrad(lambda: K.gemm_tn(dm, a["a"].view(M, D), G(blk.attn.proj.weight), G(blk.attn.proj.bias)))
             if not tail_done:
                 K.linear(dm, self.St(blk.attn.proj.weight), None, out=self.dtmp.view(M, D))
-            self._attn_bwd(l, self.dtmp)
+            self._attn_bwd(l, self.da_top if self._top_cls(l) else self.dtmp)
             self._wgrad(lambda: K.gemm_tn(dqkv.view(M, 3 * D), a["xn1"].view(M, D), G(blk.attn.qkv.weight), None))
             if self.fuse_lnbwd and self.group_wgrad and l > lo:
                 pass
@@ -742,13 +780,24 @@
             probes.append(dict(name="attn_bwd", kernel="attn_core_bwd_kernel", fns=attn_bwd, flop=2 * attn_core_flop,
                                bytes=(3 + 1 + 3) * M * D * es))
         if self.tail2 and self.group_wgrad:
+            def scr(l):
+                if not self._top_cls(l):
+                    return None
+                if self._probe_scratch is None:
+                    z = lambda *s, dt=self.T: torch.zeros(*s, dtype=dt, device=self.dev)
+                    zf = lambda *s: torch.zeros(*s, dtype=torch.float32, device=self.dev)
+                    self._probe_scratch = dict(xmid=z(B, N, D), m2=zf(M), r2=zf(M), u=z(M, hid), h=z(M, hid),
+                                               xn2=(None if self.recompute_ln else z(B, N, D)), xout=z(B, N, D),
+                                               du=z(M, hid), dxmid=z(B, N, D))
+                return self._probe_scratch
             def tail_f(l):
                 blk, a = mdl.blocks[l], self.act[l]
                 nxt = (self.act[l + 1]["m1"], self.act[l + 1]["r1"]) if l + 1 < self.Lyr else None
-                return lambda: self._block_tail_fwd(l, blk, a, nxt, save=True)
+                sc = scr(l)
+                return lambda: self._block_tail_fwd(l, blk, a, nxt, save=True, scratch=sc)
             def tail_b(l):
-                blk, a = mdl.blocks[l], self.act[l]
-                return lambda: self._block_tail_bwd(l, blk, a)
+                blk, a, sc = mdl.blocks[l], self.act[l], scr(l)
+                return lambda: self._block_tail_bwd(l, blk, a, scratch=sc)
             tail_flop = 2 * M * D * D + 2 * 2 * M * D * hid
             probes.append(dict(name="block_tail_fwd",
                                kernel="block_tail2_fwd_kernel" +
diff --git a/vit-rpe-rope_amd/vitpe/kernels.py b/vit-rpe-rope_amd/vitpe/kernels.py
--- a/vit-rpe-rope_amd/vitpe/kernels.py
+++ b/vit-rpe-rope_amd/vitpe/kernels.py
@@ -194,6 +194,43 @@
     return out, du, da
 
 
+def tail_cls_fwd(attn_out, x_in, wp_pk, bp, gamma, beta, w1_pk, b1, w2_pk, b2, B, row_step, x_mid, mean2, rstd2, out,
+                 xn_out=None, gp=None, h=None, eps2=1e-5):
+    require_device(attn_out, x_in, wp_pk, bp, gamma, beta, w1_pk, b1, w2_pk, b2, x_mid, mean2, rstd2, xn_out, gp, h, out)
+    M, D = attn_out.shape
+    HID = b1.numel()
+    assert row_step >= 1 and (B == 0 or (B - 1) * row_step < M)
+    assert x_in.shape == x_mid.shape == out.shape == (M, D) and mean2.numel() == M and rstd2.numel() == M
+    assert wp_pk.numel() == D * D and w1_pk.numel() == HID * D and w2_pk.numel() == D * HID
+    assert attn_out.dtype == x_in.dtype == wp_pk.dtype == w1_pk.dtype == w2_pk.dtype == x_mid.dtype == out.dtype
+    assert xn_out is None or (xn_out.shape == (M, D) and xn_out.dtype == attn_out.dtype)
+    assert (gp is None) == (h is None)
+    if gp is not None:
+        assert gp.shape == h.shape == (M, HID) and h.dtype == attn_out.dtype and gp.dtype == torch.float16
+    for t_, n_ in ((bp, "bp"), (gamma, "gamma"), (beta, "beta"), (b1, "b1"), (b2, "b2"), (mean2, "mean2"), (rstd2, "rstd2")):
+        _f32(t_, n_)
+    check(lib().vitpe_tail_cls_fwd(dtype_code(attn_out.dtype), ptr(attn_out), ptr(x_in), ptr(wp_pk), ptr(bp), ptr(gamma),
+                                   ptr(beta), ptr(x_mid), ptr(mean2), ptr(rstd2), ptr(xn_out), ptr(w1_pk), ptr(b1),
+                                   ptr(w2_pk), ptr(b2), ptr(gp), ptr(h), ptr(out), float(eps2), int(B), int(row_step), D, HID,
+                                   stream_ptr()), "vitpe_tail_cls_fwd")
+
+
+def tail_cls_bwd(dy, gp, w2t_pk, w1t_pk, x_mid, mean2, rstd2, gamma, dgamma, dbeta, wpt_pk, B, row_step, du, out, da):
+    require_device(dy, gp, w2t_pk, w1t_pk, x_mid, mean2, rstd2, gamma, dgamma, dbeta, wpt_pk, du, out, da)
+    M, D = dy.shape
+    HID = gp.shape[1]
+    assert row_step >= 1 and (B == 0 or (B - 1) * row_step < M)
+    assert gp.shape == du.shape == (M, HID) and x_mid.shape == out.shape == da.shape == (M, D)
+    assert mean2.numel() == M and rstd2.numel() == M and w2t_pk.numel() == HID * D and w1t_pk.numel() == HID * D
+    assert wpt_pk.numel() == D * D
+    assert dy.dtype == w2t_pk.dtype == w1t_pk.dtype == x_mid.dtype == wpt_pk.dtype == du.dtype == out.dtype == da.dtype
+    assert gp.dtype == torch.float16
+    _f32(gamma, "gamma"), _f32(dgamma, "dgamma"), _f32(dbeta, "dbeta"), _f32(mean2, "mean2"), _f32(rstd2, "rstd2")
+    check(lib().vitpe_tail_cls_bwd(dtype_code(dy.dtype), ptr(dy), ptr(gp), ptr(w2t_pk), ptr(w1t_pk), ptr(x_mid), ptr(mean2),
+                                   ptr(rstd2), ptr(gamma), ptr(du), ptr(out), ptr(dgamma), ptr(dbeta), ptr(wpt_pk), ptr(da),
+                                   int(B), int(row_step), D, HID, stream_ptr()), "vitpe_tail_cls_bwd")
+
+
 class _WgradProblem(ctypes.Structure):
     _fields_ = [("dY", ctypes.c_void_p), ("X", ctypes.c_void_p), ("dW", ctypes.c_void_p), ("dbias", ctypes.c_void_p),
                 ("M", ctypes.c_int), ("N", ctypes.c_int), ("K", ctypes.c_int), ("x_op", ctypes.c_int),
@@ -206,19 +243,24 @@
     MAX = 28
 
     def __init__(self, problems):
-        problems = [tuple(p) + (None,) * (5 - len(p)) for p in problems]
+        problems = [tuple(p) + (None,) * (6 - len(p)) for p in problems]
         if not 0 < len(problems) <= self.MAX:
             raise L.VitpeError(f"WgradGroup takes 1..{self.MAX} problems, got {len(problems)}")
-        self.keep = [p[:4] for p in problems]
+        self.keep = [(p[0][::p[5]], p[1][::p[5]]) + p[2:4] if p[5] else p[:4] for p in problems]
+        self._full = [p[:2] for p in problems]
         self._ln = [p[4] for p in problems]
         self.dtype = problems[0][0].dtype
         self.arr = (_WgradProblem * len(problems))()
-        for i, (dy, x, dw, db, ln) in enumerate(problems):
+        self.steps = (ctypes.c_int * len(problems))(*[int(p[5] or 1) for p in problems])
+        self.strided = any(st != 1 for st in self.steps)
+        for i, (dy, x, dw, db, ln, rs) in enumerate(problems):
             require_device(dy, x, dw, db)
-            M, N = dy.shape
+            rs = int(rs or 1)
+            Mfull, N = dy.shape
             K = x.shape[1]
-            assert x.shape[0] == M and dw.numel() == N * K and dy.dtype == x.dtype == self.dtype
+            assert rs >= 1 and x.shape[0] == Mfull and dw.numel() == N * K and dy.dtype == x.dtype == self.dtype
             assert dy.is_contiguous() and x.is_contiguous() and dw.is_contiguous()
+            M = -(-Mfull // rs)
             _f32(dw, "dw"), _f32(db, "dbias")
             if ln is None:
                 self.arr[i] = _WgradProblem(ptr(dy), ptr(x), ptr(dw), ptr(db), M, N, K, 0, None, None, None, None)
@@ -227,11 +269,15 @@
                 require_device(mean, rstd, gamma, beta)
                 for t_, n_ in ((mean, "mean"), (rstd, "rstd"), (gamma, "gamma"), (beta, "beta")):
                     _f32(t_, n_)
-                assert mean.numel() == M and rstd.numel() == M and gamma.numel() == K and beta.numel() == K
+                assert mean.numel() == Mfull and rstd.numel() == Mfull and gamma.numel() == K and beta.numel() == K
                 self.arr[i] = _WgradProblem(ptr(dy), ptr(x), ptr(dw), ptr(db), M, N, K, 1, ptr(mean), ptr(rstd), ptr(gamma),
                                             ptr(beta))
 
     def launch(self):
+        if self.strided:
+            check(lib().vitpe_wgrad_group_rows(dtype_code(self.dtype), ctypes.addressof(self.arr), ctypes.addressof(self.steps),
+                                               len(self.arr), stream_ptr()), "vitpe_wgrad_group_rows")
+            return
         check(lib().vitpe_wgrad_group(dtype_code(self.dtype), ctypes.addressof(self.arr), len(self.arr), stream_ptr()),
               "vitpe_wgrad_group")
 
```

Result: faster. 354,900 images/sec (median of 6 runs) (+5.3%).
